# wangkepfe/Real-Time-Ray-Tracing

Hardware: AMD Instinct MI355X
Metric: Mray/s + ms/frame at 1080p 4spp (1/2/4/8 GPU); LBVH build ms (higher is better)
Workload: dtype f32; 1 GPU; BASELINE config 3: 1920x1080, 4 spp path trace + SVGF denoise + auto-exposure/tone map, per-frame LBVH rebuild; width=1920, height=1080, spp=4

## Files before the change

### include/rtx_amd.h

```cpp
#ifndef RTX_AMD_H
#define RTX_AMD_H

#include <stddef.h>
#include <stdint.h>

#ifdef __cplusplus
extern "C" {
#endif

#define RT_OK 0
#define RT_ERR_ARG (-1)
#define RT_ERR_HIP (-2)
#define RT_ERR_IO (-3)
#define RT_ERR_STATE (-4)
#define RT_ERR_NO_DEVICE (-5)
#define RT_ERR_DEVICE (-6)

typedef struct rt_context rt_context;


int rt_create(int screen_width, int screen_height, const char* config_toml, rt_context** out);

int rt_init(rt_context* ctx);

// ... 175 lines not shown
    float emission[3];
    float ior;
    float alpha;
    float f0[3];
} rt_material;
int rt_default_material(uint32_t id, rt_material* out);
int rt_set_materials(rt_context* ctx, uint32_t first_id, uint32_t count, const rt_material* m);
int rt_get_materials(const rt_context* ctx, uint32_t first_id, uint32_t count, rt_material* out);
int rt_reset_materials(rt_context* ctx);

int rt_trace_primary(rt_context* ctx, int frame_num, int with_detail);

int rt_path_trace(rt_context* ctx, int frame_num, int with_detail);

int rt_denoise_post(rt_context* ctx, int frame_num, int with_hdr);

int rt_get_ray_count(rt_context* ctx, uint64_t* rays, int reset);

#define RT_OWN_STREAM ((void*)(intptr_t)-1)
#define RT_STREAM_OFF ((void*)(intptr_t)-2)
int rt_set_stream(rt_context* ctx, void* stream);

#define RT_GBUFFER_SETS 4
#define RT_BUF_SET1 0x100
#define RT_BUF_SET2 0x200
#define RT_BUF_SET3 0x300
int rt_set_post_stream(rt_context* ctx, void* stream);

int rt_set_gather_stream(rt_context* ctx, void* stream);

typedef struct rt_strip_exchange {
    int32_t frameNum;
    int32_t rowBegin, rowEnd;
    int32_t historySet;
    int32_t gbufferSet;
    int32_t stripLocal;
} rt_strip_exchange;
#define RT_HOOK_HISTOGRAM 0
#define RT_HOOK_ROWS 1
#define RT_HOOK_GBUFFERS 2
typedef int (*rt_collective_fn)(void* arg, int stage, void* stream, const rt_strip_exchange* x);
int rt_set_collective_hook(rt_context* ctx, rt_collective_fn fn, void* arg);
int rt_set_hook_stages(rt_context* ctx, uint32_t stage_mask);

int rt_bind_buffer(rt_context* ctx, int name, void* device_ptr, size_t bytes);

int rt_sync(rt_context* ctx);

int rt_time_stage(rt_context* ctx, int stage, int iters, float* total_ms);

int rt_time_mesh_set(rt_context* ctx, int iters, float* parts_ms);

int rt_debug_pk_math(int fn, const float* x, float y, float c, float* out_pk, float* out_scalar, size_t n);

int rt_time_path_trace_kernels(rt_context* ctx, int iters, float* kernel_ms, int n);

int rt_time_frame_kernels(rt_context* ctx, int first_frame, int iters, float* kernel_ms, int n);

int rt_frame_marks_begin(rt_context* ctx, int frames, uint32_t kernel_mask);
int rt_frame_marks_read(rt_context* ctx, float* kernel_ms, int n, int* frames_recorded);

enum rt_array_name {
    RT_ARR_VERTICES = 0,
    RT_ARR_INDICES = 1,
    RT_ARR_NORMALS = 2,
    RT_ARR_TRI_POS = 3,
    RT_ARR_AABBS = 4,
    RT_ARR_MORTON = 5,
    RT_ARR_REORDER = 6,
    RT_ARR_NODES = 7,
    RT_ARR_TLAS_AABBS = 8,
    RT_ARR_TLAS_MORTON = 9,
    RT_ARR_TLAS_REORDER = 10,
    RT_ARR_TLAS_NODES = 11,
    RT_ARR_TLAS_SCENE_AABB = 12,
    RT_ARR_BATCH_SCENE_AABBS = 13,
    RT_ARR_HITS = 14,
    RT_ARR_HIT_NORMALS = 15,
    RT_ARR_HIT_FAKE_NORMALS = 16,
    RT_ARR_HIT_STATS = 17,
    RT_ARR_TRI_NRM = 18,
    RT_ARR_RAYS = 19,
    RT_ARR_SKY_PDF = 20,
    RT_ARR_SKY_CDF = 21,
    RT_ARR_SUN_PDF = 22,
    RT_ARR_SUN_CDF = 23,
    RT_ARR_SUN_DIR = 24,
    RT_ARR_HISTOGRAM = 25,
    RT_ARR_EXPOSURE = 26,
    RT_ARR_COLOR4 = 27,
    RT_ARR_COLOR16 = 28,
    RT_ARR_COLOR64 = 29,
    RT_ARR_RGBA8 = 30,
    RT_ARR_PT_QUEUE = 32,
    RT_ARR_PT_Q3_ORIGINS = 33,
    RT_ARR_PT_Q3_DIRS = 34,
    RT_ARR_PT_Q4_ORIGINS = 35,
    RT_ARR_PT_Q4_DIRS = 36,
    RT_ARR_PT_STATS = 31,
    RT_ARR_TEX_ALBEDO_AO = 37,
    RT_ARR_TEX_NORMAL_ROUGHNESS = 38,
    RT_ARR_TEX_HEIGHT = 39,
    RT_ARR_HDR = 40,
    RT_ARR_BVH_ARENA = 41,
    RT_ARR_TRI_MATERIALS = 42,
    RT_ARR_ADJ_OFFSETS = 43,
// ... 28 lines not shown
```

### real-time-ray-tracing_amd/csrc/bvh_kernels.h

```cpp
#pragma once
#include <hip/hip_runtime.h>
#include <stdint.h>

constexpr int kStatusTlasTimeout = 0;
constexpr int kStatusTlasTimeoutBuild = 1;
constexpr int kStatusMeshBadIndices = 2;
constexpr int kStatusMatUndeclared = 3;

struct BvhBuildParams {
    const float* vertices;
    const float* normals;
    const uint32_t* indices;
    uint32_t triCount;
    uint32_t triCountPadded;
    uint32_t batchCount;
    float4* triPos;
    float4* triNrm;
    float* aabbs;
    float* batchSceneAabbs;
    uint32_t* morton;
    uint32_t* reorder;
    void* nodes;
    float* tlasAabbs;
    float* tlasSceneAabb;
    uint32_t* tlasMorton;
    uint32_t* tlasReorder;
    void* tlasNodes;
    uint32_t* counter;
    uint32_t threads;
    uint32_t cus;
    uint32_t* status;
    uint64_t waitTicks;
    uint32_t skipPublish;
    uint32_t buildSeq;
};

struct TraceCamera {
    float pos[3];
    float adjustedFront[3], adjustedLeft[3], adjustedUp[3];
    float apertureLeft[3], apertureUp[3];
    float invRes[2];
};

constexpr uint32_t kRowBlock = 16;
__host__ __device__ inline uint32_t row_of(uint32_t y0, uint32_t nStrips, uint32_t strip, uint32_t yl) {
    return y0 + ((yl / kRowBlock) * nStrips + strip) * kRowBlock + yl % kRowBlock;
}
__host__ __device__ inline uint32_t local_row(uint32_t y0, uint32_t nStrips, uint32_t y) {
    const uint32_t r = y - y0;
    return (r / kRowBlock / nStrips) * kRowBlock + r % kRowBlock;
}
inline uint32_t strip_row_count(uint32_t height, uint32_t nStrips, uint32_t strip) {
    uint32_t n = 0;
    for (uint32_t b = strip; b * kRowBlock < height; b += nStrips) {
        const uint32_t lo = b * kRowBlock, hi = lo + kRowBlock < height ? lo + kRowBlock : height;
        n += hi - lo;
    }
    return n;
}

constexpr uint32_t kDenoiseBlock = 64;
inline bool denoise_rows(uint32_t height, uint32_t nStrips, uint32_t strip, uint32_t& a, uint32_t& b) {
    const uint32_t nb = (height + kDenoiseBlock - 1) / kDenoiseBlock;
    if (nStrips < 1 || strip >= nStrips || nb < nStrips) return false;
    const uint32_t b0 = (uint32_t)((uint64_t)strip * nb / nStrips), b1 = (uint32_t)((uint64_t)(strip + 1) * nb / nStrips);
    a = b0 * kDenoiseBlock;
    b = b1 * kDenoiseBlock < height ? b1 * kDenoiseBlock : height;
    return true;
}

constexpr uint32_t kGbufHaloTiles = 5;
inline void gbuffer_rows(uint32_t height, uint32_t a, uint32_t b, uint32_t& lo, uint32_t& hi) {
    const uint32_t t0 = a / 16, t1 = (b + 15) / 16;
    lo = t0 > kGbufHaloTiles ? (t0 - kGbufHaloTiles) * 16 : 0;
    hi = (t1 + kGbufHaloTiles) * 16 < height ? (t1 + kGbufHaloTiles) * 16 : height;
}

struct TracePrimaryParams {
    TraceCamera cam;
    uint32_t width, height;
    uint32_t y0, rows;
    uint32_t nStrips, strip;
    int frameNum;
    const uint8_t* bluenoise;
    const float4* triPos;
    const float4* triNrm;
    const void* nodes;
    const void* tlasNodes;
    float4* hitOut;
    float4* normalOut;
    float4* fakeNormalOut;
    uint32_t* statsOut;
};

struct GeomUpdateParams {
    const float* src;
    uint32_t first, count;
    float* vertices;
    float* normals;
    const uint32_t* indices;
    const uint32_t* cornerSlot;
    const uint32_t* adjOffsets;
    float* contrib;
    uint32_t nverts, triCountPadded;
    float* prevVerts;
};

struct GeomDispParams {
    const float* vertices;
    const float* prevVerts;
    const uint32_t* indices;
    float4* triDisp;
    uint32_t triCountPadded;
};

constexpr uint32_t kMeshSortThreads = 512;
constexpr uint32_t kMeshTilesMax = 256;
inline uint32_t mesh_tile_len(uint32_t corners) {
    const uint32_t per = (corners + kMeshTilesMax - 1) / kMeshTilesMax;
    return (per + kMeshSortThreads - 1) / kMeshSortThreads * kMeshSortThreads;
}
struct MeshSetParams {
    const uint32_t* srcIndices;
    uint32_t triCount, triCountPadded, nverts;
    uint32_t* indices;
    uint32_t* adjOffsets;
    uint32_t* adjCorner;
    uint32_t* cornerSlot;
    uint32_t* keys[2];
    uint32_t* vals[2];
    uint32_t* table;
    uint32_t* badCount;
    uint32_t* status;
};
extern "C" hipError_t rtk_launch_mesh_set(const MeshSetParams* p, hipStream_t stream, hipEvent_t afterIngest);

extern "C" hipError_t rtk_launch_geometry_update(const GeomUpdateParams* p, hipStream_t stream);
// ... 7 lines not shown
```

### real-time-ray-tracing_amd/csrc/context.cpp

```cpp
#include "context.h"

#include <dlfcn.h>
#include <stdio.h>
#include <string.h>

#include <algorithm>
#include <chrono>
#include <cmath>
#include <fstream>
#include <sstream>

#include "gaussian_tables.h"
#include "mat_kernels.h"
#include "rtmath.h"
#include "toml_lite.h"

namespace {

thread_local std::string g_createError;

void default_params(rt_params& p) {
    p.sky.needRegenerate = 1;
    p.sky.timeOfDay = 0.25f;
    p.sky.sunAxisAngle = 45.0f;
// ... 1131 lines not shown
    }
    if (!ctx->dMatTable) {
        if (int rc = dalloc(ctx, &ctx->dMatTable, 256 * sizeof(MatRecord))) return rc;
    }
    HIP_TRY(ctx, hipMemcpy(ctx->dMatTable, recs.data(), 256 * sizeof(MatRecord), hipMemcpyHostToDevice));
    ctx->matHost.swap(next);
    ctx->matCustom = true;
    ctx->matEmits = emits;
    ++ctx->matSerial;
    return RT_OK;
}

int rt_get_materials(const rt_context* ctx, uint32_t first_id, uint32_t count, rt_material* out) {
    if (!ctx || !out) return RT_ERR_ARG;
    if (count == 0u || (uint64_t)first_id + (uint64_t)count > 256u) return RT_ERR_ARG;
    for (uint32_t k = 0; k < count; ++k) {
        if (ctx->matCustom) out[k] = ctx->matHost[first_id + k];
        else (void)rt_default_material(first_id + k, &out[k]);
    }
    return RT_OK;
}

int rt_reset_materials(rt_context* ctx) {
    if (!ctx) return RT_ERR_ARG;
    if (!ctx->inited) { ctx->err = "rt_reset_materials before rt_init"; return RT_ERR_STATE; }
    if (int rc = sync_streams(ctx, false)) return rc;
    ctx->matCustom = false;
    ctx->matEmits = false;
    ++ctx->matSerial;
    return RT_OK;
}

int wait_bvh(rt_context* ctx) {
    if (ctx->buildOnSide[ctx->bvhSet])
        HIP_TRY(ctx, hipStreamWaitEvent(ctx->stream, ctx->buildDone[ctx->bvhSet], 0));
    return RT_OK;
}

int rt_trace_primary(rt_context* ctx, int frame_num, int with_detail) {
    if (!ctx) return RT_ERR_ARG;
    if (!ctx->inited) { ctx->err = "rt_trace_primary before rt_init"; return RT_ERR_STATE; }
    HostCamera hc;
    rt_camera_update(ctx->camera, ctx->renderW, ctx->renderH, hc);
    TracePrimaryParams p;
    p.cam = rt_trace_camera(hc);
    p.width = (uint32_t)ctx->renderW;
    p.height = (uint32_t)ctx->renderH;
    p.y0 = (uint32_t)ctx->stripY0;
    p.rows = (uint32_t)ctx->stripRows;
    p.nStrips = (uint32_t)ctx->stripCount;
    p.strip = (uint32_t)ctx->stripIndex;
    p.frameNum = frame_num;
    p.bluenoise = ctx->dBlueNoise;
    p.triPos = ctx->dTriPos;
    p.triNrm = ctx->dTriNrm;
    p.nodes = ctx->dNodes;
    p.tlasNodes = ctx->dTlasNodes;
    p.hitOut = ctx->dHits;
    p.normalOut = with_detail ? ctx->dHitNrm : nullptr;
    p.fakeNormalOut = with_detail ? ctx->dHitFake : nullptr;
    p.statsOut = with_detail ? ctx->dHitStats : nullptr;
    if (int rc = wait_bvh(ctx)) return rc;
    HIP_TRY(ctx, rtk_launch_trace_primary(&p, ctx->stream));
    return RT_OK;
}

int rt_sync(rt_context* ctx) {
    if (!ctx) return RT_ERR_ARG;
    if (!ctx->inited) return RT_OK;
    return sync_streams(ctx);
}

int rt_draw_frame_internal(rt_context* ctx);

int rt_time_stage(rt_context* ctx, int stage, int iters, float* total_ms) {
    if (!ctx || !total_ms || iters < 1) return RT_ERR_ARG;
    if (!ctx->inited) { ctx->err = "rt_time_stage before rt_init"; return RT_ERR_STATE; }
    if (ctx->postStream) {
        void* post = ctx->postStream;
        int rc = rt_set_post_stream(ctx, nullptr);
        if (rc == RT_OK) rc = rt_time_stage(ctx, stage, iters, total_ms);
        const int rc2 = rt_set_post_stream(ctx, post);
        return rc != RT_OK ? rc : rc2;
    }
    const MeshChange same{ctx->dIdxStage, ctx->mesh.triCount, ctx->nv};
    if (stage == 5 || stage == 6) {
        int rc = sync_streams(ctx, false);
        if (rc == RT_OK) rc = vertex_stage(ctx);
        if (rc != RT_OK) return rc;
        HIP_TRY(ctx, hipMemcpy(ctx->dVertStage, ctx->dVerts, (size_t)ctx->nv * 12, hipMemcpyDeviceToDevice));
        if (stage == 6)
            HIP_TRY(ctx, hipMemcpy(ctx->dIdxStage, ctx->dIdx, (size_t)ctx->mesh.triCount * 12, hipMemcpyDeviceToDevice));
        HIP_TRY(ctx, hipDeviceSynchronize());
    }
    HIP_TRY(ctx, hipEventRecord(ctx->ev0, ctx->stream));
    for (int i = 0; i < iters; ++i) {
        int rc = RT_OK;
        if (stage == 0) rc = rt_build_bvh(ctx);
        else if (stage == 5) rc = enqueue_vertex_update(ctx, ctx->dVertStage, 0, ctx->nv, nullptr, true, false);
        else if (stage == 6) rc = enqueue_vertex_update(ctx, ctx->dVertStage, 0, ctx->nv, nullptr, true, false, &same);
        else if (stage == 1) rc = rt_trace_primary(ctx, 1 + i, 0);
        else if (stage == 2) rc = rt_path_trace(ctx, 1 + i, 0);
        else if (stage == 3) {
            const int f = ctx->nextFrame++;
            if ((rc = rt_build_bvh(ctx)) == RT_OK && (rc = rt_path_trace(ctx, f, 0)) == RT_OK)
                rc = rt_denoise_post(ctx, f, 0);
// ... 305 lines not shown
```

### real-time-ray-tracing_amd/csrc/context.h

```cpp
#pragma once
#include <hip/hip_runtime.h>
#include <stdint.h>

#include <string>
#include <vector>

#include "../../include/rtx_amd.h"
#include "bvh_kernels.h"
#include "frame_kernels.h"
#include "scene_gen.h"
#include "soil_textures.h"

struct HostCamera {
    float pos[3], dir[3], left[3], up[3];
    float yaw, pitch, focal, aperture;
    float res[2], invRes[2], fov[2], tanHalfFov[2];
    float adjustedLeft[3], adjustedUp[3], adjustedFront[3], apertureLeft[3], apertureUp[3];
};

inline size_t arena_bytes(size_t B, size_t NP) { return (B * 1024 + B + NP) * 64; }

struct BvhBufs {
    float4* triPos = nullptr;
    float4* triNrm = nullptr;
    float* aabbs = nullptr;
    float* batchScene = nullptr;
    uint32_t* morton = nullptr;
    uint32_t* reorder = nullptr;
    void* nodes = nullptr;
    float* tlasAabbs = nullptr;
    float* tlasScene = nullptr;
    uint32_t* tlasMorton = nullptr;
    uint32_t* tlasReorder = nullptr;
    void* tlasNodes = nullptr;
    uint32_t* counter = nullptr;
    float4* triDisp = nullptr;
    uint32_t triCount = 0, triCountPadded = 0, B = 0;
    uint64_t meshSerial = 0;
};

#ifndef RTX_GB_SETS
#define RTX_GB_SETS RT_GBUFFER_SETS
#endif
constexpr int kGbSets = RTX_GB_SETS;

constexpr int kMatPool = 4;

struct FrameResources {
    bool ready = false;
    float* solar = nullptr;
    float* limb = nullptr;
    float* cie = nullptr;
    float4* sky = nullptr;
    float* skyPdf = nullptr;
    float* skyCdf = nullptr;
    float4* sun = nullptr;
    float* sunPdf = nullptr;
    float* sunCdf = nullptr;
    float* scanSums = nullptr;
    float* skyTree = nullptr;
    float* sunTree = nullptr;
    float* lightSel = nullptr;
    bool skyValid = false;
    rt_sky_params lastSky{};
    float sunDir[3] = {0, 1, 0};
    float cosThetaMax = 1.0f, sunArea = 0.0f;
    uint2* texAlbedo = nullptr;
    uint2* texNormal = nullptr;
    uint16_t* texHeight = nullptr;
    uint2* gColor[kGbSets] = {};
    uint2* gNormal[kGbSets] = {};
    uint2* gAlbedo[kGbSets] = {};
    uint16_t* gDepth[kGbSets] = {};
    uint32_t* gMotion[kGbSets] = {};
    int gbSet = 0;
    bool setInFlight[kGbSets] = {};
    uint2* color = nullptr;
    uint2* normal = nullptr;
    uint2* albedo = nullptr;
    uint16_t* depth = nullptr;
    uint32_t* motion = nullptr;
    uint32_t* rays = nullptr;
    uint4* ptStats = nullptr;
    unsigned long long* rayCounter = nullptr;
    PtWorkspace ws{};
    float4* camHit0Rec[kGbSets] = {};
    float* camHit0Err[kGbSets] = {};
    uint32_t* camSurface[kGbSets] = {};
    uint32_t* camCount[kGbSets] = {};
    uint32_t* lastCounters = nullptr;
    uint32_t* syncCount[3] = {};
    int syncIdx = 0;
    bool syncZeroed[3] = {};
    struct Spec {
        bool valid = false;
        bool shade = false;
        int block = 0;
        uint64_t epoch = 0;
        uint64_t matSerial = 0;
        PathTraceParams p{};
    } spec;
    bool specReady = false;
    bool gbBound = false;
    unsigned long long* specRayCounter = nullptr;
    int specCounts = 0;
    bool camInFlight[kGbSets] = {};
    PtQueue camQ3[kGbSets] = {}, camQ4[kGbSets] = {};
    float4* camHitRec[kGbSets] = {};
    float* camHitErr[kGbSets] = {};
    float4* camPathL[kGbSets] = {};
    uint32_t* camPending[kGbSets] = {};
    uint32_t* camShade3[kGbSets] = {};
    int lastSlot = 0;
    unsigned long long* q3Host = nullptr;
// ... 261 lines not shown
```

### real-time-ray-tracing_amd/csrc/debug_math.hip

```cpp
#include <hip/hip_runtime.h>

#include "rtmath_pk.h"
#include "rtx_amd.h"

namespace {
__global__ __launch_bounds__(256) void k_debug_pk(int fn, const float* x, float y, float c, float* outPk,
                                                  float* outScalar, size_t n) {
    const size_t i = (size_t)blockIdx.x * 256 + threadIdx.x;
    if (i >= n) return;
    const size_t j = (i ^ 1) < n ? (i ^ 1) : i;
    const rtpk::F2 v = {x[i], x[j]};
    float pk = 0.0f, sc = 0.0f;
    if (fn == 0) {
        pk = rtpk::pow_pos2(v, y, rtpk::pow_y_odd(y)).x;
        sc = rt_powf(x[i], y);
    } else if (fn == 1) {
        pk = rtpk::expf2(v).x;
        sc = rt_expf(x[i]);
    } else {
        pk = rtpk::div_rcp2(v, y, c).x;
        sc = rt_div_rcp(x[i], y, c);
    }
    outPk[i] = pk;
    outScalar[i] = sc;
}
}

extern "C" int rt_debug_pk_math(int fn, const float* x, float y, float c, float* out_pk, float* out_scalar, size_t n) {
    if (!x || !out_pk || !out_scalar || fn < 0 || fn > 2) return RT_ERR_ARG;
    if (fn == 0 && !(y > 0.0f && y < __builtin_inff())) return RT_ERR_ARG;
    if (n == 0) return RT_OK;
    hipLaunchKernelGGL(k_debug_pk, dim3((unsigned)((n + 255) / 256)), dim3(256), 0, 0, fn, x, y, c, out_pk, out_scalar, n);
    if (hipGetLastError() != hipSuccess || hipDeviceSynchronize() != hipSuccess) return RT_ERR_HIP;
    return RT_OK;
}
```

### real-time-ray-tracing_amd/csrc/frame.cpp

```cpp
#include <math.h>
#include <stdlib.h>
#include <string.h>

#include <chrono>
#include <fstream>
#include <utility>
#include <vector>

#include "context.h"
#include "rtmath.h"

namespace {

constexpr float kPi = 3.1415926535897932384626422832795028841971f;
constexpr float kTwoPi = 6.2831853071795864769252867665590057683943f;
constexpr float kPiOver180 = 0.01745329251f;

struct V3 { float x, y, z; };
V3 v3(float x, float y, float z) { return V3{x, y, z}; }
V3 operator+(V3 a, V3 b) { return v3(a.x + b.x, a.y + b.y, a.z + b.z); }
V3 operator*(V3 a, float s) { return v3(a.x * s, a.y * s, a.z * s); }
V3 operator*(float s, V3 a) { return v3(a.x * s, a.y * s, a.z * s); }
V3 operator-(V3 a) { return v3(-a.x, -a.y, -a.z); }
float dop(float a, float b, float c, float d) {
// ... 17 lines not shown
    const float n = sqrtf(v.x * v.x + v.y * v.y + v.z * v.z);
    return v3(v.x / n, v.y / n, v.z / n);
}

struct Quat { V3 v; float w; };
Quat qmul(const Quat& p, const Quat& q) { return Quat{p.w * q.v + q.w * p.v + cross(p.v, q.v), p.w * q.w - dot(p.v, q.v)}; }

V3 sun_direction(float timeOfDay, float sunAxisAngle) {
    const V3 axis = normalize(v3(0.0f, rt_cosf(sunAxisAngle * kPiOver180), rt_sinf(sunAxisAngle * kPiOver180)));
    const float angle = fmodf(timeOfDay * kPi, kTwoPi);
    const V3 v = cross(v3(0.0f, 1.0f, 0.0f), axis);
    const Quat q{normalize(axis) * rt_sinf(angle / 2), rt_cosf(angle / 2)};
    const Quat r = qmul(qmul(q, Quat{v, 0.0f}), Quat{-q.v, q.w});
    return normalize(r.v);
}

float fitting(const float* m, float s, int i) {
    return (rt_powf(1.0f - s, 5.0f) * m[i] + 5.0f * rt_powf(1.0f - s, 4.0f) * s * m[i + 9] +
            10.0f * rt_powf(1.0f - s, 3.0f) * rt_powf(s, 2.0f) * m[i + 18] +
            10.0f * rt_powf(1.0f - s, 2.0f) * rt_powf(s, 3.0f) * m[i + 27] +
            5.0f * (1.0f - s) * rt_powf(s, 4.0f) * m[i + 36] + rt_powf(s, 5.0f) * m[i + 45]);
}
float fitting2(const float* m, float s) {
    return (rt_powf(1.0f - s, 5.0f) * m[0] + 5.0f * rt_powf(1.0f - s, 4.0f) * s * m[1] +
            10.0f * rt_powf(1.0f - s, 3.0f) * rt_powf(s, 2.0f) * m[2] +
            10.0f * rt_powf(1.0f - s, 2.0f) * rt_powf(s, 3.0f) * m[3] + 5.0f * (1.0f - s) * rt_powf(s, 4.0f) * m[4] +
            rt_powf(s, 5.0f) * m[5]);
}

struct SkyTablesHost {
    std::vector<float> skyDataSets, skyDataSetsRad, solar, limb, cieX, cieY, cieZ;
};
SkyTablesHost g_tables;

bool load_sky_tables(const std::string& path, SkyTablesHost& t, std::string& err) {
    std::ifstream f(path, std::ios::binary);
    if (!f) { err = "cannot read " + path; return false; }
    uint32_t count = 0;
    f.read((char*)&count, 4);
    if (count != 7) { err = "bad sky table file " + path; return false; }
    uint32_t len[7];
    f.read((char*)len, sizeof(len));
    const uint32_t expect[7] = {540, 60, 1800, 60, 10, 10, 10};
    std::vector<float>* dst[7] = {&t.skyDataSets, &t.skyDataSetsRad, &t.solar, &t.limb, &t.cieX, &t.cieY, &t.cieZ};
    for (int i = 0; i < 7; ++i) {
        if (len[i] != expect[i]) { err = "bad sky table sizes in " + path; return false; }
        dst[i]->resize(len[i]);
        f.read((char*)dst[i]->data(), len[i] * 4);
    }
    if (!f) { err = "truncated " + path; return false; }
    return true;
}

bool sky_params_equal(const rt_sky_params& a, const rt_sky_params& b) {
    return a.timeOfDay == b.timeOfDay && a.sunAxisAngle == b.sunAxisAngle && a.skyScalar == b.skyScalar &&
           a.sunScalar == b.sunScalar && a.sunAngle == b.sunAngle;
}

int update_sky(rt_context* ctx) {
    FrameResources& fr = ctx->fr;
    rt_sky_params& sp = ctx->params.sky;
    const V3 sunDir = sun_direction(sp.timeOfDay, sp.sunAxisAngle);
    fr.sunDir[0] = sunDir.x; fr.sunDir[1] = sunDir.y; fr.sunDir[2] = sunDir.z;
    if (fr.skyValid && !sp.needRegenerate && sky_params_equal(sp, fr.lastSky)) return RT_OK;
    if (fr.spec.valid) HIP_TRY(ctx, hipStreamWaitEvent(ctx->stream, ctx->specDone, 0));
    if (ctx->postStream) {
        const int rc = sync_streams(ctx, false);
        if (rc != RT_OK) return rc;
    }
    sp.sunScalar = sp.sunScalar > 0.00001f ? sp.sunScalar : 0.00001f;
    sp.skyScalar = sp.skyScalar > 0.00001f ? sp.skyScalar : 0.00001f;
    sp.sunAngle = sp.sunAngle > 0.51f ? sp.sunAngle : 0.51f;
    SkyGenParams p;
    memcpy(p.sunDir, fr.sunDir, 12);
    p.skyScalar = sp.skyScalar;
    p.sunScalar = sp.sunScalar;
    p.sunAngle = sp.sunAngle;
    const float elevation = rt_acosf(sunDir.y);
    const float se = rt_powf(elevation / (kPi / 2.0f), (1.0f / 3.0f));
    for (int ch = 0; ch < 10; ++ch) {
        for (int i = 0; i < 9; ++i) p.st.configs[ch * 9 + i] = fitting(g_tables.skyDataSets.data() + ch * 54, se, i);
        p.st.radiances[ch] = fitting2(g_tables.skyDataSetsRad.data() + ch * 6, se);
    }
    const float sunRadius = sp.sunAngle * kPi / 180.0f / 2.0f;
    p.cosThetaMax = rt_cosf(sunRadius);
    p.solar = fr.solar;
    p.limb = fr.limb;
    p.cie = fr.cie;
    p.skyBuffer = fr.sky;
    p.skyPdf = fr.skyPdf;
    p.skyCdf = fr.skyCdf;
    p.sunBuffer = fr.sun;
    p.sunPdf = fr.sunPdf;
    p.sunCdf = fr.sunCdf;
    p.scanSums = fr.scanSums;
    p.skyTree = fr.skyTree;
    p.sunTree = fr.sunTree;
    p.lightSel = fr.lightSel;
    HIP_TRY(ctx, rtk_launch_sky(&p, ctx->stream));
    if (ctx->postStream) HIP_TRY(ctx, hipStreamSynchronize(ctx->stream));
    fr.sunArea = rt_powf(rt_tanf(sunRadius), 2.0f) * kPi;
    fr.cosThetaMax = p.cosThetaMax;
    fr.skyValid = true;
    sp.needRegenerate = 0;
    fr.lastSky = sp;
    return RT_OK;
}

float dop_host(float a, float b, float c, float d) {
    const float cd = c * d;
    const float err = fmaf(-c, d, cd);
    const float dp = fmaf(a, b, -cd);
    return dp + err;
}
void sun_frame(const float n[3], float t[3], float b[3]) {
    float w[3] = {1.0f, 0.0f, 0.0f};
    if (fabsf(n[0]) > 0.707f) { w[0] = 0.0f; w[1] = 1.0f; }
    auto cross = [](const float* a, const float* c, float* r) {
        r[0] = dop_host(a[1], c[2], a[2], c[1]);
        r[1] = dop_host(a[2], c[0], a[0], c[2]);
        r[2] = dop_host(a[0], c[1], a[1], c[0]);
    };
    cross(n, w, t);
    cross(n, t, b);
}

HistCamera hist_of(const HostCamera& c) {
    HistCamera h;
    memcpy(h.pos, c.pos, 12);
    memcpy(h.left, c.left, 12);
    memcpy(h.up, c.up, 12);
    memcpy(h.dir, c.dir, 12);
    return h;
}

}

void select_gbuffers(FrameResources& fr) {
    const int k = fr.gbSet;
    if (fr.renderColor == fr.color) fr.renderColor = fr.gColor[k];
    fr.color = fr.gColor[k];
    fr.normal = fr.gNormal[k];
    fr.albedo = fr.gAlbedo[k];
    fr.depth = fr.gDepth[k];
    fr.motion = fr.gMotion[k];
}

bool strip_local_denoise(const rt_context* ctx, uint32_t& a, uint32_t& b) {
    const rt_render_pass_settings& ps = ctx->params.pass;
    const uint32_t H = (uint32_t)ctx->renderH;
    a = 0;
// ... 152 lines not shown
}

float frame_delta(rt_context* ctx) {
    FrameResources& fr = ctx->fr;
    if (fr.drawDt >= 0.0f) {
        const float d = fr.drawDt;
        fr.drawDt = -1.0f;
        return d;
    }
    if (ctx->deltaMs > 0.0f) return ctx->deltaMs;
    const double now = std::chrono::duration<double>(std::chrono::steady_clock::now().time_since_epoch()).count();
    const float dt = fr.lastDrawTime < 0 ? 1000.0f / 60.0f : (float)((now - fr.lastDrawTime) * 1000.0);
    fr.lastDrawTime = now;
    return dt;
}

void update_dynamic_resolution(rt_context* ctx, float dt) {
    if (!(dt > 0.0f)) return;
    const float hi = 1000.0f / (ctx->targetFps - 2), lo = 1000.0f / (ctx->targetFps + 2);
    int w = ctx->renderW;
    if (hi < dt || lo > dt) {
        const float ratio = sqrtf((1000.0f / ctx->targetFps) / dt);
        w = (int)((float)w * ratio);
    }
    w = w + ((w % 16 < 8) ? (-w % 16) : (16 - w % 16));
    w = w < ctx->minWidth ? ctx->minWidth : w > ctx->maxWidth ? ctx->maxWidth : w;
    int h = (w / 16) * 9;
    if (h > ctx->maxHeight) h = ctx->maxHeight;
    ctx->renderW = w;
    ctx->renderH = h;
    ctx->stripRows = h;
}

int rt_frame_init(rt_context* ctx) {
    FrameResources& fr = ctx->fr;
    std::string err;
    if (g_tables.solar.empty()) {
        SkyTablesHost t;
        if (!load_sky_tables(rt_data_dir() + "/sky_tables.bin", t, err)) { ctx->err = err; return RT_ERR_IO; }
        g_tables = std::move(t);
    }
    int rc;
#define ALLOC(p, bytes) if ((rc = dalloc(ctx, &(p), (bytes))) != RT_OK) return rc
    ALLOC(fr.solar, 1800 * 4);
    ALLOC(fr.limb, 60 * 4);
    ALLOC(fr.cie, 30 * 4);
    ALLOC(fr.sky, (size_t)kSkySize * 16);
    ALLOC(fr.skyPdf, (size_t)kSkySize * 4);
    ALLOC(fr.skyCdf, (size_t)kSkySize * 4);
    ALLOC(fr.sun, (size_t)kSunSize * 16);
    ALLOC(fr.sunPdf, (size_t)kSunSize * 4);
    ALLOC(fr.sunCdf, (size_t)kSunSize * 4);
    ALLOC(fr.scanSums, 512 * 4);
    ALLOC(fr.skyTree, (size_t)kSkyTreeNodes * 4);
    ALLOC(fr.sunTree, (size_t)kSunTreeNodes * 4);
    ALLOC(fr.lightSel, 16);
    ALLOC(fr.texAlbedo, (size_t)kTexTexels * 8);
    ALLOC(fr.texNormal, (size_t)kTexTexels * 8);
    ALLOC(fr.texHeight, (size_t)kTexTexels * 2);
    HIP_TRY(ctx, hipMemset(fr.texHeight, 0, (size_t)kTexTexels * 2));
    const size_t P = (size_t)ctx->renderW * ctx->renderH;
    ALLOC(fr.color, P * 8);
    ALLOC(fr.normal, P * 8);
    ALLOC(fr.albedo, P * 8);
    ALLOC(fr.depth, P * 2);
    ALLOC(fr.motion, P * 4);
    fr.gColor[0] = fr.color;
    fr.gNormal[0] = fr.normal;
    fr.gAlbedo[0] = fr.albedo;
    fr.gDepth[0] = fr.depth;
    fr.gMotion[0] = fr.motion;
    ALLOC(fr.rays, P * 4);
    ALLOC(fr.ptStats, P * 16);
    ALLOC(fr.rayCounter, (size_t)kRayCounterSlots * kRayCounterStride * 8);
    {
        const size_t cap = (size_t)ctx->renderW * ctx->stripRows * ctx->spp;
        if (cap >= (1ull << 31)) { ctx->err = "strip x spp too large for the path-trace queues"; return RT_ERR_ARG; }
        PtWorkspace& ws = fr.ws;
        ws.cap = (uint32_t)cap;
        ALLOC(ws.hit0Rec, cap * 16);
        ALLOC(ws.hit0Err, cap * 4);
        for (PtQueue* q : {&ws.q3, &ws.q4}) {
            ALLOC(q->rayO, cap * 16);
            ALLOC(q->rayD, cap * 16);
            ALLOC(q->st0, cap * 16);
            ALLOC(q->st1, cap * 16);
            ALLOC(q->st2, cap * 16);
        }
        ALLOC(ws.hitRec, cap * 16);
        ALLOC(ws.hitErr, cap * 4);
        ALLOC(ws.pathL, cap * 16);
        if (ctx->tune.resumeSplit > 0) ALLOC(fr.camShade3[0], cap * 4);
        ALLOC(ws.pending, (size_t)ctx->renderW * ctx->stripRows * 4);
        ALLOC(ws.surface, (size_t)ctx->renderW * ctx->stripRows * 4);
        ALLOC(fr.camCount[0], kWsCounterWords * 4);
        ALLOC(fr.syncCount[1], kWsCounterWords * 4);
        ALLOC(fr.syncCount[2], kWsCounterWords * 4);
        fr.syncCount[0] = fr.camCount[0];
        fr.camQ3[0] = ws.q3;
        fr.camQ4[0] = ws.q4;
        fr.camHitRec[0] = ws.hitRec;
        fr.camHitErr[0] = ws.hitErr;
        fr.camPathL[0] = ws.pathL;
        fr.camPending[0] = ws.pending;
        fr.camHit0Rec[0] = ws.hit0Rec;
        fr.camHit0Err[0] = ws.hit0Err;
        fr.camSurface[0] = ws.surface;
        ws.counters = fr.camCount[0];
        ws.fetch = ws.counters + 64;
// ... 126 lines not shown
    if (queues) {
        for (PtQueue* q : {&fr.camQ3[k], &fr.camQ4[k]}) {
            ALLOC(q->rayO, cap * 16);
            ALLOC(q->rayD, cap * 16);
            ALLOC(q->st0, cap * 16);
            ALLOC(q->st1, cap * 16);
            ALLOC(q->st2, cap * 16);
        }
        ALLOC(fr.camHitRec[k], cap * 16);
        ALLOC(fr.camHitErr[k], cap * 4);
        ALLOC(fr.camPathL[k], cap * 16);
        ALLOC(fr.camPending[k], strip * 4);
        if (ctx->tune.resumeSplit > 0) ALLOC(fr.camShade3[k], cap * 4);
    }
#undef ALLOC
    return rc;
}

int fill_pt_params(const rt_context* ctx, int frame_num, int with_detail, const HostCamera& hc, int g,
                   PathTraceParams& p) {
    const FrameResources& fr = ctx->fr;
    memset(&p, 0, sizeof p);
    p.cam = rt_trace_camera(hc);
    p.tanHalfFov[0] = hc.tanHalfFov[0];
    p.tanHalfFov[1] = hc.tanHalfFov[1];
    p.res[0] = hc.res[0];
    p.res[1] = hc.res[1];
    p.halfRes[0] = hc.res[0] / 2;
    p.halfRes[1] = hc.res[1] / 2;
    p.hist = fr.hist;
    p.width = (uint32_t)ctx->renderW;
    p.height = (uint32_t)ctx->renderH;
    p.y0 = (uint32_t)ctx->stripY0;
    p.rows = (uint32_t)ctx->stripRows;
    p.nStrips = (uint32_t)ctx->stripCount;
    p.strip = (uint32_t)ctx->stripIndex;
    p.frameNum = frame_num;
    p.spp = (uint32_t)ctx->spp;
    p.invSpp = (ctx->spp & (ctx->spp - 1)) == 0 ? 1.0f / (float)ctx->spp : 0.0f;
    p.materialOverride = ctx->materialOverride;
    p.triCount = ctx->bvh[ctx->bvhSet].triCount;
    p.bluenoise = ctx->dBlueNoise;
    p.triPos = ctx->dTriPos;
    p.triNrm = ctx->dTriNrm;
    p.triDisp = ctx->dispValid[ctx->bvhSet] && !ctx->dispTraced[ctx->bvhSet] ? ctx->bvh[ctx->bvhSet].triDisp : nullptr;
    p.nodes = ctx->dNodes;
    p.tlasNodes = ctx->dTlasNodes;
    p.texAlbedo = fr.texAlbedo;
    p.texNormal = fr.texNormal;
    p.skyBuffer = fr.sky;
    p.sunBuffer = fr.sun;
    p.skyCdf = fr.skyCdf;
    p.sunCdf = fr.sunCdf;
    p.skyTree = fr.skyTree;
    p.sunTree = fr.sunTree;
    p.lightSel = fr.lightSel;
    memcpy(p.sunDir, fr.sunDir, 12);
    p.cosThetaMax = fr.cosThetaMax;
    p.oneMinusCosThetaMax = 1.0f - fr.cosThetaMax;
    sun_frame(fr.sunDir, p.sunT, p.sunB);
    p.colorOut = fr.gColor[g];
    p.normalOut = fr.gNormal[g];
    p.albedoOut = fr.gAlbedo[g];
    p.depthOut = fr.gDepth[g];
    p.motionOut = fr.gMotion[g];
    p.raysOut = with_detail ? fr.rays : nullptr;
    p.statsOut = with_detail ? fr.ptStats : nullptr;
    p.rayCounter = fr.rayCounter;
    p.ws = fr.ws;
    p.ws.hit0Rec = fr.camHit0Rec[g];
    p.ws.hit0Err = fr.camHit0Err[g];
    p.ws.surface = fr.camSurface[g];
    p.ws.counters = fr.camCount[g];
    p.ws.fetch = p.ws.counters + 64;
    const int qs = fr.camQ3[g].rayO ? g : 0;
    p.ws.q3 = fr.camQ3[qs];
    p.ws.q4 = fr.camQ4[qs];
    p.ws.hitRec = fr.camHitRec[qs];
    p.ws.hitErr = fr.camHitErr[qs];
    p.ws.pathL = fr.camPathL[qs];
    p.ws.pending = fr.camPending[qs];
    p.ws.hitRec4 = p.ws.hitRec;
    p.ws.hitErr4 = p.ws.hitErr;
    p.ws.shade3 = fr.camShade3[qs];
    {
        const int m = ctx->materialOverride;
        uint32_t classes = ctx->dTriMat ? ctx->triMatClasses : 0u;
        if (m >= 0) {
            const uint8_t id = (uint8_t)(m > 255 ? 255 : m);
            (void)rt_material_classes(&id, 1, &classes);
        }
        p.triMat = m >= 0 ? nullptr : ctx->dTriMat;
        p.ws.glossy = (classes & RT_MAT_CLASS_GLOSSY) != 0u;
        p.ws.microfacet = (classes & RT_MAT_CLASS_MICROFACET) != 0u;
        p.matTable = ctx->matCustom ? reinterpret_cast<const float4*>(ctx->dMatTable) : nullptr;
        if (p.matTable) p.ws.glossy = p.ws.microfacet = 1;
        p.ws.closest4 = p.matTable && ctx->matEmits ? 1 : 0;
    }
    return qs;
}

bool spec_on(const rt_context* ctx) {
    return ctx->tune.syncSpec && ctx->fr.specReady && !ctx->postStream && ctx->stripCount == 1 && !ctx->fr.gbBound;
}

bool spec_matches(const PathTraceParams& a, uint64_t epochA, uint64_t matA, const PathTraceParams& b, uint64_t epochB,
                  uint64_t matB) {
    if (epochA != epochB) return false;
    if (matA != matB) return false;
// ... 838 lines not shown
    HIP_TRY(ctx, hipMemsetAsync(fr.ws.counters, 0, kWsCounterWords * sizeof(uint32_t), ctx->stream));
    HIP_TRY(ctx, hipMemcpyAsync(fr.ws.counters + kCntQ3, &n, 4, hipMemcpyHostToDevice, ctx->stream));
    HIP_TRY(ctx, hipEventRecord(ctx->ev0, ctx->stream));
    HIP_TRY(ctx, rtk_launch_trace_queue(&p, 3, ctx->stream));
    HIP_TRY(ctx, hipEventRecord(ctx->ev1, ctx->stream));
    HIP_TRY(ctx, hipMemcpyAsync(hits, fr.ws.hitRec, (size_t)n * 16, hipMemcpyDeviceToHost, ctx->stream));
    if (iters) HIP_TRY(ctx, hipMemcpyAsync(iters, p.ws.itersOut, (size_t)n * 4, hipMemcpyDeviceToHost, ctx->stream));
    HIP_TRY(ctx, hipStreamSynchronize(ctx->stream));
    if (kernel_ms) HIP_TRY(ctx, hipEventElapsedTime(kernel_ms, ctx->ev0, ctx->ev1));
    return RT_OK;
}

int rt_trace_rays_device(rt_context* ctx, const rt_ray_query* q) {
    if (!ctx || !q) return RT_ERR_ARG;
    const char* bad = nullptr;
    if (q->org_stride < 3u || q->dir_stride < 3u) bad = "strides are in floats and at least 3";
    else if (q->n > RT_QUERY_MAX_RAYS) bad = "more rays than RT_QUERY_MAX_RAYS";
    else if ((q->flags & ~RT_QUERY_ANY_HIT) != 0u) bad = "unknown flags";
    else if (q->n > 0u && (!q->org || !q->dir || !q->hits)) bad = "org, dir and hits must not be NULL";
    else if (((uintptr_t)q->hits & 15u) != 0) bad = "hits must be 16-byte aligned";
    else if ((((uintptr_t)q->org | (uintptr_t)q->dir | (uintptr_t)q->iters) & 3u) != 0) bad = "org, dir and iters must be 4-byte aligned";
    if (bad) { ctx->err = std::string("rt_trace_rays_device: ") + bad; return RT_ERR_ARG; }
    if (!ctx->inited) { ctx->err = "rt_trace_rays_device before rt_init"; return RT_ERR_STATE; }
    hipStream_t s = ctx->stream;
    if (q->n > 0u) {
        if (q->ready_event) HIP_TRY(ctx, hipStreamWaitEvent(s, (hipEvent_t)q->ready_event, 0));
        if (int rc = wait_bvh(ctx)) return rc;
        RayQueryParams p;
        p.nodes = ctx->dNodes;
        p.tlasNodes = ctx->dTlasNodes;
        p.triPos = ctx->dTriPos;
        p.org = q->org;
        p.dir = q->dir;
        p.orgStride = q->org_stride;
        p.dirStride = q->dir_stride;
        p.n = q->n;
        p.hits = reinterpret_cast<float4*>(q->hits);
        p.iters = q->iters;
        p.fetch = ctx->queryFetch;
        HIP_TRY(ctx, hipMemsetAsync(ctx->queryFetch, 0, 512, s));
        HIP_TRY(ctx, rtk_launch_trace_rays(&p, ctx->fr.ws.traceBlocks, (q->flags & RT_QUERY_ANY_HIT) != 0u, s));
        const int k = ctx->bvhSet;
        if (ctx->postStream) {
            HIP_TRY(ctx, hipEventRecord(ctx->bvhFree[k], s));
            ctx->bvhInFlight[k] = true;
        } else {
            HIP_TRY(ctx, hipEventRecord(ctx->queryDone[k], s));
            ctx->queryInFlight[k] = true;
        }
    }
    if (q->done_event) HIP_TRY(ctx, hipEventRecord((hipEvent_t)q->done_event, s));
    return RT_OK;
}
```

### real-time-ray-tracing_amd/csrc/frame_kernels.h

```cpp
#pragma once
#include <hip/hip_runtime.h>
#include <stdint.h>

#include "bvh_kernels.h"
#include "rtx_amd.h"

constexpr int kSkyW = 512, kSkyH = 256, kSkySize = kSkyW * kSkyH;
constexpr int kSunW = 32, kSunH = 32, kSunSize = kSunW * kSunH;
constexpr int kSkyScanBlock = 256, kSunScanBlock = 32;
constexpr int kTexLevels = 11, kTexSize = 1024;

static_assert((kTexSize & (kTexSize - 1)) == 0 && kTexSize <= 16384, "power-of-two texture size");
__host__ __device__ constexpr uint32_t tex_level_offset(int l) {
    return 4u * ((uint32_t)(kTexSize * kTexSize) - (uint32_t)(kTexSize >> l) * (uint32_t)(kTexSize >> l)) / 3u;
}
constexpr uint32_t kTexTexels = tex_level_offset(kTexLevels);

struct SkyState {
    float configs[90];
    float radiances[10];
};

struct SkyGenParams {
    float sunDir[3];
    float skyScalar, sunScalar, sunAngle;
    float cosThetaMax;
    SkyState st;
    const float* solar;
    const float* limb;
    const float* cie;
    float4* skyBuffer;
    float* skyPdf;
    float* skyCdf;
    float4* sunBuffer;
    float* sunPdf;
    float* sunCdf;
    float* scanSums;
    float* skyTree;
    float* sunTree;
    float* lightSel;
};

constexpr int kSkyTreeNodes = 4096, kSunTreeNodes = 1024;

struct HistCamera { float pos[3], left[3], up[3], dir[3]; };

constexpr uint32_t kQShadowFlag = 1u;

__host__ __device__ inline bool q3_shades(uint32_t flags, uint32_t hitIdxBits) {
    return (flags & kQShadowFlag) == 0u && (int32_t)hitIdxBits >= 0;
}

struct PtQueue {
    float4* rayO;
    float4* rayD;
    float4* st0;
    float4* st1;
    float4* st2;
};

enum PtCounter : int { kCntQ3 = 0, kCntQ4 = 1, kCntFetch3 = 2, kCntFetch4 = 3, kCntPending = 4, kCntResume3 = 5,
                       kCntResume4 = 6, kCntResolve = 7, kCntMaxIter3 = 8, kCntMaxIter4 = 9, kCntError = 10,
                       kCntSurface = 11, kCntVisCam = 12, kCntTstCam = 13, kCntVisShade = 14, kCntTstShade = 15,
                       kCntVisQ3 = 16, kCntTstQ3 = 17, kCntVisQ4 = 18, kCntTstQ4 = 19, kCntDiffShade = 20,
                       kCntDiffRes3 = 21, kCntCulledCam = 22, kCntShade3 = 23, kCntSlots = 24 };
constexpr int kWsCounterWords = 64 + 3 * 8 * 16;
constexpr uint32_t kChainMaxQ3 = 1u << 20;

struct PtWorkspace {
    float4* hit0Rec;
    float* hit0Err;
    PtQueue q3, q4;
    float4* hitRec;
    float* hitErr;
    float4* hitRec4 = nullptr;
    float* hitErr4 = nullptr;
    uint32_t* shade3 = nullptr;
    float4* pathL;
    uint32_t* pending;
    uint32_t* surface;
    uint32_t* counters;
    uint32_t* fetch;
    uint32_t cap;
    uint32_t persistBlocks;
    int shadeClaim = 0;
    uint32_t shadeBlocksPerCu = 0;
    uint32_t cus = 256;
    uint32_t traceBlocks;
    uint32_t trace3ShortBlocks = 0;
    uint32_t trace4Blocks;
    int glossy;
    int microfacet;
    int chain = 1;
    int closest4 = 0;
    uint32_t* itersOut = nullptr;
    unsigned long long* q3HostOut = nullptr;
    uint32_t q3Tag = 0;
    uint32_t* zeroNext = nullptr;
    int countersZeroed = 0;
};

enum class PtBouncePlan { chain, split, unsplit };
inline PtBouncePlan pt_bounce_plan(const PtWorkspace& ws) {
    if (ws.chain && !ws.glossy && !ws.microfacet) return PtBouncePlan::chain;
    return ws.shade3 && !ws.glossy ? PtBouncePlan::split : PtBouncePlan::unsplit;
}

constexpr int kRayCounterSlots = 256, kRayCounterStride = 16;

struct PathTraceParams {
    TraceCamera cam;
    float tanHalfFov[2];
    float res[2];
    float halfRes[2];
    HistCamera hist;
    uint32_t width, height;
    uint32_t y0, rows;
    uint32_t nStrips, strip;
    int frameNum;
    uint32_t spp;
    float invSpp;
    int materialOverride;
    uint32_t triCount;
    const uint8_t* bluenoise;
    const float4* triPos;
    const float4* triNrm;
    const void* nodes;
    const void* tlasNodes;
    const uint2* texAlbedo;
    const uint2* texNormal;
    const float4* skyBuffer;
    const float4* sunBuffer;
    const float* skyCdf;
    const float* sunCdf;
    const float* skyTree;
    const float* sunTree;
    const float* lightSel;
    float sunDir[3];
    float sunT[3], sunB[3];
    float cosThetaMax;
    float oneMinusCosThetaMax;
    uint2* colorOut;
    uint2* normalOut;
    uint2* albedoOut;
    uint16_t* depthOut;
    uint32_t* motionOut;
    uint32_t* raysOut;
    uint4* statsOut;
    unsigned long long* rayCounter;
    PtWorkspace ws;
    const float4* triDisp;
    const uint8_t* triMat;
    const float4* matTable;
};

constexpr int kMatRecVecs = 4;
struct alignas(16) MatRecord {
    float color[3];
    uint32_t typeFlags;
    float f0[3];
    float alpha;
    float emission[3];
    float ior;
    float pad[4];
};
static_assert(sizeof(MatRecord) == 16 * kMatRecVecs, "four 16-byte vectors");

struct DenoisePostParams {
    uint32_t W, H;
    uint32_t Ws, Hs;
    uint32_t histW, histH;
    int frameNum;
    float deltaTime;
    int temporal, localSpatial, visualize, wideSpatial, temporal2;
    int postProcess, downScale, histogramOn, autoExposure, sharpen, tonemap;
    int bloom, lensFlare;
    int toneMappingType;
    float sunPos[2];
    int sunUv[2];
    uint2* bloom4;
    uint2* bloom16;
    float gain, fixedExposure, maxWhite, gamma;
    rt_denoising_params dn;
    uint2* colorA;
    uint2* colorB;
    uint2* normal;
    const uint2* albedo;
    uint16_t* depth;
    const uint32_t* motion;
    uint2* accum;
    uint2* accumAlt;
    uint2* histColor;
    uint2* histColorOut;
    uint16_t* histDepth;
    uint16_t* noise8;
    uint16_t* noise16;
    uint2* c4;
    uint2* c16;
    uint2* c64;
    uint32_t* histogram;
    float* exposure;
    uint2* scaledA;
    uint2* scaledB;
    uint32_t* rgba;
    uint32_t rgbaPitch;
    const uint8_t* bluenoise;
    float4* hdrOut;
    uint2* finalColor;
    uint2* finalScaled;
    int stripLocal;
    uint32_t rowA, rowB;
    int histOutSet;
    int gbSet;
    uint32_t* rgbaTarget;
    uint32_t rgbaTargetPitch;
    int ty0, ty1;
    int cty0, cty1;
    uint32_t* chainCounter;
    int exposureDone;
    int histDepthInTemporal;
    uint2* svgfOut;
    int histDepthDone;
    uint32_t* tileList;
    uint32_t tileCap;
    int tileParity;
    int listUsed;
    int listSplit;
    int listFold;
    float rcpDepth[3];
    int rcpDepthOk;
    hipEvent_t* marks;
};
constexpr int kDnKernels = 8;

extern "C" hipError_t rtk_denoise_post(DenoisePostParams* p, hipStream_t stream);
extern "C" hipError_t rtk_denoise_phase(DenoisePostParams* p, hipStream_t stream, int phase);
extern "C" hipError_t rtk_hdr_out(const uint2* color, float4* hdr, size_t n, hipStream_t stream);

extern "C" hipError_t rtk_launch_sky(const SkyGenParams* p, hipStream_t stream);
extern "C" hipError_t rtk_launch_mipgen(uint16_t* chain, int size, int levels, int channels, hipStream_t stream);
extern "C" hipError_t rtk_launch_scan(const float* in, float* out, float* sums, int size, int blockSize,
                                      hipStream_t stream);
extern "C" hipError_t rtk_launch_scan_ex(const float* in, float* out, float* sums, int size, int blockSize,
                                         int postfix, hipStream_t stream);
constexpr int kPtKernels = 7;
constexpr int kFrameKernels = kPtKernels + kDnKernels;
struct PtLaunchHook {
    hipError_t (*fn)(void* arg, int kernel);
    void* arg;
};
struct PtLeanFork {
    hipStream_t stream;
    hipEvent_t traced, done;
};
extern "C" hipError_t rtk_launch_pt_camera(const PathTraceParams* p, hipStream_t stream, hipEvent_t* marks);
extern "C" hipError_t rtk_launch_pt_rest(const PathTraceParams* p, hipStream_t stream, hipEvent_t* marks,
                                         const PtLaunchHook* hook, const PtLeanFork* fork);
extern "C" hipError_t rtk_launch_pt_shade(const PathTraceParams* p, hipStream_t stream, hipEvent_t* marks);
extern "C" hipError_t rtk_fold_ray_counts(unsigned long long* dst, unsigned long long* src, hipStream_t stream);
extern "C" hipError_t rtk_launch_pt_rest_after_shade(const PathTraceParams* p, hipStream_t stream, hipEvent_t* marks,
                                                     const PtLaunchHook* hook, const PtLeanFork* fork);
extern "C" int rtk_trace_queue_blocks_per_cu();
extern "C" hipError_t rtk_launch_trace_queue(const PathTraceParams* p, int step, hipStream_t stream);

struct RayQueryParams {
    const void* nodes;
    const void* tlasNodes;
    const float4* triPos;
    const float* org;
    const float* dir;
    uint32_t orgStride, dirStride;
    uint32_t n;
    float4* hits;
    uint32_t* iters;
    uint32_t* fetch;
};
extern "C" hipError_t rtk_launch_trace_rays(const RayQueryParams* p, uint32_t maxBlocks, int anyHit, hipStream_t stream);
```

### real-time-ray-tracing_amd/csrc/pathtrace.hip

```cpp
#include "frame_kernels.h"
#include "pt_common.h"
#include "queue_fetch.h"
#include "shade.h"
#include "traverse.h"

using namespace rtd;

namespace {

constexpr uint32_t kQShadow = kQShadowFlag;
constexpr int kQSampleShift = 1;
constexpr int kQLightShift = 16;

struct RayState {
    F3 orig, dir, pos, normal, fakeNormal, albedo, centerRaydir;
    int matId, matType, lightIdx, objectIdx;
    bool isRayIntoSurface, hitLight, hit, isDiffuse, isHitProcessed, isOccluded, isShadowRay;
    float offset, normalDotRayDir, depth, rayConeWidth, rayConeSpread;
};

struct PathCtx {
    const PathTraceParams& P;
    F3 sunDir;
    const uint32_t* sob;
    BnPixel bp;
    int frameIdx;
    uint32_t rays, visits, tests, diffuse;
    const float* skyTree = nullptr;
    const float* sunTree = nullptr;
};

RT_DEV PathCtx path_ctx(const PathTraceParams& P, const uint32_t* sob, const float* skyTree, const float* sunTree) {
    return PathCtx{P, f3(P.sunDir[0], P.sunDir[1], P.sunDir[2]), sob, BnPixel{0u, 0u}, 0, 0u, 0u, 0u, 0u, skyTree, sunTree};
}

RT_DEV void stage_cdf_trees(const PathTraceParams& P, float* sky, float* sun, int tid, int nthreads) {
    for (int i = tid; i < kSkyTreeNodes / 4; i += nthreads) reinterpret_cast<float4*>(sky)[i] = reinterpret_cast<const float4*>(P.skyTree)[i];
    for (int i = tid; i < kSunTreeNodes / 4; i += nthreads) reinterpret_cast<float4*>(sun)[i] = reinterpret_cast<const float4*>(P.sunTree)[i];
}

RT_DEV float rnd(const PathCtx& c, int k, int d) { return bn_value(c.sob, c.bp, c.frameIdx * 4 + k, d); }

struct PathVars {
    RayState rs;
    F3 beta0, beta1;
    float outDepth;
    uint32_t mask;
    F2 mv, sampleUv;
    F3 outNormal;
};

RT_DEV float4 mat_vec(const PathTraceParams& P, int id, int k) { return P.matTable[(id & 255) * kMatRecVecs + k]; }

template <bool kTab = false>
RT_DEV void update_material(const PathTraceParams& P, RayState& rs) {
    const bool inRange = rs.objectIdx >= 0 && rs.objectIdx < (int)P.triCount;
    int tableId = 3;
    if (P.triMat && inRange) tableId = (int)P.triMat[rs.objectIdx];
    const int id = P.materialOverride >= 0 ? P.materialOverride : inRange ? tableId : 6;
    int type;
    if constexpr (kTab) type = (int)(__float_as_uint(mat_vec(P, id, 0).w) & 0xFFu);
    else type = (id >= 0 && id < 10) ? mat_type(id) : PERFECT_REFLECTION;
    rs.matId = rs.hit ? id : 99999;
    rs.matType = rs.hit ? type : MAT_SKY;
    if (rs.isShadowRay) {
        if ((rs.matType == EMISSIVE && rs.lightIdx == rs.objectIdx) || (rs.matType == MAT_SKY && rs.lightIdx == kEnvLightId))
            rs.hitLight = true;
        else
            rs.isOccluded = true;
    } else {
        rs.hitLight = rs.matType == EMISSIVE || rs.matType == MAT_SKY;
    }
    rs.isDiffuse = (rs.matType == LAMBERTIAN) || (rs.matType == MICROFACET);
}

RT_DEV bool needs_trace(const RayState& rs) { return !(rs.hitLight || !rs.isHitProcessed || rs.isOccluded); }

template <bool kTab = false>
RT_DEV void apply_hit(const PathTraceParams& P, RayState& rs, const HitInfo& h) {
    rs.isHitProcessed = false;
    rs.offset = h.offset;
    rs.objectIdx = h.objectIdx;
    rs.pos = h.pos;
    rs.normal = h.normal;
    rs.fakeNormal = h.fakeNormal;
    rs.normalDotRayDir = h.ndr;
    rs.isRayIntoSurface = h.into;
    rs.hit = h.hit;
    rs.depth = h.t;
    if (rs.hit) rs.rayConeWidth += rs.rayConeSpread * h.t;
    update_material<kTab>(P, rs);
}

template <bool kTab = false>
// ... 36 lines not shown
RT_DEV void tri_plane(const PathTraceParams& P, F2 uv, float lod, F3 normal, F3 w, F3& alb, F3& nrm) {
    uv.x *= 0.5f;
    uv.y *= 0.5f;
    const F4 t0 = sample_lod(P.texAlbedo, uv, lod);
    __builtin_amdgcn_sched_barrier(0);
    alb = f3(rt_powf_div(t0.x, 2.2f), rt_powf_div(t0.y, 2.2f), rt_powf_div(t0.z, 2.2f));
    __builtin_amdgcn_sched_barrier(0);
    const F4 t1 = sample_lod(P.texNormal, uv, lod);
    const F3 n = f3(t1.x - 0.5f, t1.y - 0.5f, t1.z - 0.5f);
    const F3 u = cross(normal, w);
    const F3 v = cross(normal, u);
    nrm = normalize(u * n.x + v * n.y + normal * n.z);
}

template <bool kMF, bool kTab = false>
RT_DEV void diffuse(PathCtx& c, int bounce, RayState& rs, F3& beta) {
    if (rs.hitLight || !rs.isDiffuse || rs.isOccluded) return;
    const PathTraceParams& P = c.P;
    ++c.diffuse;
    rs.lightIdx = kDefaultLightId;
    rs.isHitProcessed = true;
    F3 normal = rs.fakeNormal;
    const F3 surfaceNormal = rs.normal;
    F3 albedo;
    bool flat = false;
    if constexpr (kTab) flat = ((__float_as_uint(mat_vec(P, rs.matId, 0).w) >> 8) & RT_MAT_FLAG_FLAT) != 0u;
    if (!flat) {
        const float lod = rt_log2f_div(rs.rayConeWidth * 0.5f * __builtin_sqrtf(1024.0f * 1024.0f + 1024.0f * 1024.0f));
        const float wx = surfaceNormal.x * surfaceNormal.x, wy = surfaceNormal.y * surfaceNormal.y,
                    wz = surfaceNormal.z * surfaceNormal.z;
        F3 accA = f3(0.0f), accN = f3(0.0f);
#pragma unroll 1
        for (int pl = 0; pl < 3; ++pl) {
            const F2 uv = pl == 0 ? F2{rs.pos.y, rs.pos.z} : pl == 1 ? F2{rs.pos.x, rs.pos.z} : F2{rs.pos.x, rs.pos.y};
            F3 wv;
            if (pl == 0) wv = fabsf(normal.y) > 0.999f ? f3(0, 0, 1) : f3(0, 1, 0);
            else if (pl == 1) wv = fabsf(normal.x) > 0.999f ? f3(0, 0, 1) : f3(1, 0, 0);
            else wv = fabsf(normal.y) > 0.999f ? f3(1, 0, 0) : f3(0, 1, 0);
            F3 a, n;
            tri_plane(P, uv, lod, normal, wv, a, n);
            const float wgt = pl == 0 ? wx : pl == 1 ? wy : wz;
            accA = pl == 0 ? a * wgt : accA + a * wgt;
            accN = pl == 0 ? n * wgt : accN + n * wgt;
        }
        albedo = accA;
        normal = normalize(accN);
        rs.fakeNormal = normal;
    }
    if constexpr (kTab) {
        const float4 m0 = mat_vec(P, rs.matId, 0);
        albedo = flat ? f3(m0.x, m0.y, m0.z) : albedo * f3(m0.x, m0.y, m0.z);
    }
    if (bounce == 0) rs.albedo = albedo * (1.0f + fabsf(dot(normal, rs.centerRaydir)));
    float r[4], r2[4];
#pragma unroll
    for (int d = 0; d < 4; ++d) {
        r[d] = rnd(c, 2 * bounce, d);
        r2[d] = rnd(c, 2 * bounce + 1, d);
    }
    const F3 rayDir = rs.dir;
    F3 lDir;
    float lPdf = 1.0f;
    int lIdx;
    sample_light(P, c.sunDir, lDir, lPdf, lIdx, r2[0], r2[1], c.skyTree, c.sunTree);
    F3 sDir, sBsdf, lBsdf, tmp;
    float sPdf = 0.0f;
    if (!kMF || rs.matType == LAMBERTIAN) {
        lambertian_sample(F2{r[0], r[1]}, sDir, normal);
        sBsdf = f3(div_pi(albedo.x), div_pi(albedo.y), div_pi(albedo.z));
        sPdf = div_pi(fmx(dot(sDir, normal), kSafeCos));
        lBsdf = sBsdf;
    } else {
        F3 F0 = mat_F0(rs.matId);
        float alpha = mat_alpha(rs.matId);
        if constexpr (kTab) {
            const float4 m1 = mat_vec(P, rs.matId, 1);
            F0 = f3(m1.x, m1.y, m1.z);
            alpha = m1.w;
        }
        const float alpha2 = alpha * alpha;
        const F3 sn = ggx_normal(F2{r[0], r[1]}, alpha2, normal);
        sDir = normalize(reflect3(rayDir, sn));
        if (dot(sDir, surfaceNormal) < 0.0f) {
            const F3 sn2 = ggx_normal(F2{r[2], r[3]}, alpha2, normal);
            sDir = normalize(reflect3(rayDir, sn2));
            if (dot(sDir, surfaceNormal) < 0.0f) sDir = normalize(reflect3(rayDir, normal));
        }
        float lsPdf;
        microfacet_terms(-rayDir, sDir, sn, normal, F0, albedo, alpha2, tmp, sBsdf, sPdf);
        microfacet_terms(-rayDir, lDir, normalize(lDir + -rayDir), normal, F0, albedo, alpha2, tmp, lBsdf, lsPdf);
    }
    if (isnan3(lBsdf)) lBsdf = f3(0.0f);
    if (isnan3(sBsdf)) sBsdf = f3(0.0f);
    if (sPdf != sPdf) sPdf = 0.0f;
    if (lPdf != lPdf) lPdf = 0.0f;
    const float ph = (sPdf * sPdf) / (sPdf * sPdf + lPdf * lPdf);
    const float minPdf = 1e-5f;
    if (r[3] < ph) {
        if (dot(rs.normal, sDir) < 0.0f) { rs.isOccluded = true; return; }
        const float cwi = fmx(kSafeCos, dot(sDir, normal));
        beta = sBsdf * cwi / fmx(sPdf, minPdf);
        rs.dir = sDir;
    } else {
        if (dot(rs.normal, lDir) < 0.0f) { rs.isOccluded = true; return; }
        const float cwi = fmx(kSafeCos, dot(lDir, normal));
        beta = lBsdf * cwi / fmx(lPdf, minPdf);
        rs.dir = lDir;
        rs.lightIdx = lIdx;
        rs.isShadowRay = true;
    }
    if (isnan3(beta)) beta = f3(0.0f);
    rs.orig = rs.pos + rs.offset * rs.normal;
}

RT_DEV float ray_cone_width(const PathTraceParams& P, int ix, int iy) {
    const F2 pc = {((float)ix + 0.5f) - P.halfRes[0], ((float)iy + 0.5f) - P.halfRes[1]};
    const F2 po = {copysignf(0.5f, pc.x), copysignf(0.5f, pc.y)};
    const F2 un = {(pc.x - po.x) * P.cam.invRes[0] * 2, (pc.y - po.y) * P.cam.invRes[1] * 2};
    const F2 uf = {(pc.x + po.x) * P.cam.invRes[0] * 2, (pc.y + po.y) * P.cam.invRes[1] * 2};
    const F2 pn = {un.x * P.tanHalfFov[0], un.y * P.tanHalfFov[1]};
    const F2 pf = {uf.x * P.tanHalfFov[0], uf.y * P.tanHalfFov[1]};
    const float an = rt_atanf(__builtin_sqrtf(pn.x * pn.x + pn.y * pn.y));
    const float af = rt_atanf(__builtin_sqrtf(pf.x * pf.x + pf.y * pf.y));
    return af - an;
}

RT_DEV void gbuffer_step0(const PathCtx& c, PathVars& v) {
    const RayState& rs = v.rs;
    v.outDepth = rs.depth;
    v.mask = (uint32_t)rs.matId & 0xFFFFu;
    F2 mv = {0.0f, 0.0f};
    if (rs.hit) {
        const PathTraceParams& P = c.P;
        const F3 d = rs.pos - load3(P.hist.pos);
        const F3 q = f3(dot(load3(P.hist.left), d), dot(load3(P.hist.up), d), dot(load3(P.hist.dir), d));
        const F2 s = {q.x / q.z, q.y / q.z};
        const F2 ndc = {s.x / P.tanHalfFov[0], s.y / P.tanHalfFov[1]};
        mv = F2{(0.5f - ndc.x * 0.5f) - v.sampleUv.x, (0.5f - ndc.y * 0.5f) - v.sampleUv.y};
    }
    v.mv = F2{mv.x + 0.5f, mv.y + 0.5f};
}

template <int kDeferFrom, bool kMF, bool kTab = false>
RT_DEV int run_path(PathCtx& c, PathVars& v, int k0, const HitInfo* hit, const SceneView& sc, uint2* stk) {
    RayState& rs = v.rs;
    if (hit) apply_hit<kTab>(c.P, rs, *hit);
#pragma unroll 1
    for (int k = k0; k < 5; ++k) {
        if ((k != k0 || !hit) && needs_trace(rs)) {
            if (k >= kDeferFrom) return k;
            ++c.rays;
// ... 81 lines not shown
    const uint32_t flags = (rs.isShadowRay ? kQShadow : 0u) | (s << kQSampleShift) |
                           ((uint32_t)rs.lightIdx << kQLightShift);
    q.rayO[slot] = make_float4(rs.orig.x, rs.orig.y, rs.orig.z, __uint_as_float(pixel));
    q.rayD[slot] = make_float4(rs.dir.x, rs.dir.y, rs.dir.z, __uint_as_float(flags));
    q.st0[slot] = make_float4(rs.albedo.x, rs.albedo.y, rs.albedo.z, rs.rayConeWidth);
    q.st1[slot] = make_float4(v.beta1.x, v.beta1.y, v.beta1.z, rs.rayConeSpread);
    q.st2[slot] = make_float4(v.beta0.x, v.beta0.y, v.beta0.z, 0.0f);
}

RT_DEV SceneView scene_of(const PathTraceParams& P) { return scene_view(P.nodes, P.tlasNodes, P.triPos, P.triNrm); }

template <bool kBits = false>
RT_DEV void add_rays(const PathTraceParams& P, unsigned long long* wgSlots, uint32_t rays, int w) {
    if (!P.rayCounter) return;
    uint32_t r = rays;
    if (kBits) {
        r = (uint32_t)__popcll(__ballot(rays != 0u));
    } else {
#pragma unroll
        for (int o = 32; o > 0; o >>= 1) r += __shfl_xor(r, o);
    }
    const bool lane0 = __lane_id() == 0;
    if (lane0) wgSlots[w] = r;
    __syncthreads();
    const uint32_t slot = (blockIdx.y * gridDim.x + blockIdx.x) % kRayCounterSlots;
    if (w == 0 && lane0)
        atomicAdd(&P.rayCounter[slot * kRayCounterStride], wgSlots[0] + wgSlots[1] + wgSlots[2] + wgSlots[3]);
}
template <bool kBits = false>
RT_DEV void add_rays(const PathTraceParams& P, unsigned long long* wgSlots, uint32_t rays) {
    add_rays<kBits>(P, wgSlots, rays, __builtin_amdgcn_readfirstlane((int)threadIdx.x >> 6));
}

RT_DEV void start_sample(PathCtx& c, PathVars& v, int x, int y, float coneSpread, F3 centerDir) {
    RayState& rs = v.rs;
    v.beta0 = f3(1.0f);
    v.beta1 = f3(1.0f);
    rs.hitLight = false;
    rs.lightIdx = kDefaultLightId;
    rs.isHitProcessed = true;
    rs.isOccluded = false;
    rs.isShadowRay = false;
    rs.isDiffuse = false;
    rs.hit = false;
    rs.matType = MAT_SKY;
    rs.matId = 0;
    rs.objectIdx = -1;
    rs.normal = f3(0.0f, -1.0f, 0.0f);
    rs.fakeNormal = f3(0.0f);
    rs.albedo = f3(1.0f);
    rs.rayConeWidth = 0.0f;
    rs.rayConeSpread = coneSpread;
    rs.centerRaydir = centerDir;
    generate_ray_jittered(c.P.cam, x, y, F2{rnd(c, 0, 0), rnd(c, 0, 1)}, F2{rnd(c, 0, 2), rnd(c, 0, 3)}, rs.orig,
                          rs.dir, v.sampleUv);
    v.outDepth = 0.0f;
    v.mask = 0u;
    v.mv = F2{0.0f, 0.0f};
    v.outNormal = f3(0.0f);
}

}

__host__ __device__ inline int cam_sample_waves(uint32_t spp) { return spp >= 4 ? 4 : (spp >= 2 ? 2 : 1); }
inline bool one_round(uint32_t spp) { return spp >= 1 && ((int)spp + cam_sample_waves(spp) - 1) / cam_sample_waves(spp) == 1; }

template <bool kOneRound, bool kStats>
__global__ __launch_bounds__(256, kOneRound ? 6 : 4) void k_pt_camera(PathTraceParams P) {
    constexpr int kCamLds = 10;
    __shared__ uint2 stk[kCamLds * 256];
    __shared__ uint32_t sob[256];
    __shared__ float4 fold[4][64];
    __shared__ uint32_t surf[4][64];
    __shared__ unsigned long long wgRays[4];
    const int tid = threadIdx.x, lane = tid & 63, w = tid >> 6;
    bn_stage_sobol(P.bluenoise, sob, tid, 256);
    __syncthreads();
    const int nSW = cam_sample_waves(P.spp);
    const int sw = w % nSW, g = w / nSW, tilesX = nSW == 4 ? 1 : 2;
    const int BW = 8 * tilesX, BH = nSW == 1 ? 16 : 8;
    const int x = blockIdx.x * BW + (g % tilesX) * 8 + (lane & 7);
    const int yl = blockIdx.y * BH + (g / tilesX) * 8 + (lane >> 3);
    const bool active = x < (int)P.width && yl < (int)P.rows;
    const int y = (int)row_of(P.y0, P.nStrips, P.strip, (uint32_t)yl);
    const uint32_t p = (uint32_t)y * P.width + (uint32_t)x;
    const uint32_t pl = (uint32_t)yl * P.width + (uint32_t)x;
    const size_t plane = (size_t)P.rows * P.width;
    const SceneView sc = scene_of(P);
    PathCtx c = path_ctx(P, sob, nullptr, nullptr);
    if (active) c.bp = bn_pixel(P.bluenoise, x, y);
    const int rounds = kOneRound ? 1 : ((int)P.spp + nSW - 1) / nSW;
    F3 L = f3(0.0f), A = f3(0.0f);
    bool anyHit = false;
    float4 rec = make_float4(0.0f, 0.0f, 0.0f, 0.0f);
    float recErr = 0.0f;
    uint32_t rays = 0, camV = 0, camT = 0, camCull = 0;
#pragma unroll 1
    for (int r = 0; r < rounds; ++r) {
        const int s = r * nSW + sw;
        float4 out = make_float4(0.0f, 0.0f, 0.0f, 0.0f);
        if (active && s < (int)P.spp) {
            c.frameIdx = (int)P.spp * (P.frameNum - 1) + 1 + s;
            F3 org, dir;
            F2 uv;
            generate_ray_jittered(P.cam, x, y, F2{rnd(c, 0, 0), rnd(c, 0, 1)}, F2{rnd(c, 0, 2), rnd(c, 0, 3)}, org,
                                  dir, uv);
            TravState st;
            if (root_surely_missed(sc, org, dir)) {
                trav_root_miss(st, sc.root);
                ++camCull;
            } else {
                TravRay tr;
                trav_setup(sc, org, dir, tr);
                trav_init(st, sc.root);
                DeepStack deep;
                TravRec trec;
                for (int it = 0; it < 1024; ++it)
                    if (trav_step<kCamLds, false, kStats>(sc, tr, st, trec, stk + tid, 256, &deep)) break;
            }
            ++rays;
            if (P.statsOut) {
                camV += st.visits;
                camT += st.tests;
            }
            rec = make_float4(st.t, __uint_as_float((uint32_t)st.hitIdx), st.hitU, st.hitV);
            recErr = st.hitErrT;
            if (rounds > 1) {
                P.ws.hit0Rec[(size_t)s * plane + pl] = rec;
                P.ws.hit0Err[(size_t)s * plane + pl] = recErr;
            }
            if (st.t < kRayMax) {
                out.w = 1.0f;
            } else {
                PathVars v;
                v.rs.dir = dir;
                v.rs.hitLight = true;
                v.rs.isOccluded = false;
                v.rs.matType = MAT_SKY;
                v.rs.albedo = f3(1.0f);
                v.beta0 = f3(1.0f);
                v.beta1 = f3(1.0f);
                const F3 Ls = finish(c, v);
                out = make_float4(Ls.x, Ls.y, Ls.z, 0.0f);
            }
        }
        fold[w][lane] = out;
        __syncthreads();
        if (sw == 0 && active) {
#pragma unroll 1
            for (int k = 0; k < nSW; ++k) {
                const int sk = r * nSW + k;
                if (sk >= (int)P.spp) break;
                const float4 o = fold[g * nSW + k][lane];
                anyHit = anyHit || o.w != 0.0f;
                if (P.spp == 1) {
                    L = f3(o.x, o.y, o.z);
                    A = f3(1.0f);
                } else {
                    L = L + f3(o.x, o.y, o.z);
// ... 42 lines not shown
    add_rays<kOneRound>(P, wgRays, rays);
}

struct ShadeClaim {
    uint32_t batches, partLen, drained, next;
    int home;
    bool dyn;
};
RT_DEV void claim_init(ShadeClaim& c, uint32_t batches, bool dyn) {
    c.batches = batches;
    c.partLen = (batches + kParts - 1) / kParts;
    c.drained = batches == 0u ? (1u << kParts) - 1u : 0u;
    c.home = (int)(blockIdx.x % kParts);
    c.dyn = dyn;
    c.next = blockIdx.x;
}
RT_DEV uint32_t claim_next(ShadeClaim& c, uint32_t* counters, uint32_t& slot) {
    if (!c.dyn) {
        const uint32_t b = c.next;
        c.next += gridDim.x;
        return b;
    }
    __syncthreads();
    if (threadIdx.x == 0) {
        uint32_t b = c.batches;
        while (c.drained != (1u << kParts) - 1u) {
            int part = c.home;
            while (c.drained & (1u << part)) part = (part + 1) % kParts;
            const uint32_t got = atomicAdd(&counters[part * 16], 1u);
            const uint32_t lo = (uint32_t)part * c.partLen;
            const uint32_t len = lo >= c.batches ? 0u : (c.batches - lo < c.partLen ? c.batches - lo : c.partLen);
            if (got < len) {
                b = lo + got;
                break;
            }
            c.drained |= 1u << part;
        }
        slot = b;
    }
    __syncthreads();
    return slot;
}

template <bool kGlossy, bool kMF, bool kOneRound, bool kTab = false>
#ifndef RTX_SHADE_WAVES
#define RTX_SHADE_WAVES 3
#endif
__global__ __launch_bounds__(256, (kGlossy || !kOneRound) ? 2 : RTX_SHADE_WAVES) void k_pt_shade0(PathTraceParams P) {
    __shared__ uint2 stk[kGlossy ? 17 * 256 : 1];
    __shared__ uint32_t sob[256];
    __shared__ float4 foldL[4][64];
    __shared__ float4 foldA[4][64];
    __shared__ unsigned long long wgRays[4];
    __shared__ __align__(16) float sSkyTree[kSkyTreeNodes];
    __shared__ __align__(16) float sSunTree[kSunTreeNodes];
    __shared__ uint32_t wgBatch;
    const int tid = threadIdx.x, lane = tid & 63, w = tid >> 6;
    const int wS = __builtin_amdgcn_readfirstlane(w);
    bn_stage_sobol(P.bluenoise, sob, tid, 256);
    stage_cdf_trees(P, sSkyTree, sSunTree, tid, 256);
    __syncthreads();
    const uint32_t n = P.ws.counters[kCntSurface];
    const int nSW = cam_sample_waves(P.spp), sw = w % nSW, g = w / nSW;
    const uint32_t perWg = 64u * (uint32_t)(4 / nSW);
    const int rounds = kOneRound ? 1 : ((int)P.spp + nSW - 1) / nSW;
    const SceneView sc = scene_of(P);
    const size_t plane = (size_t)P.rows * P.width;
    uint32_t raysWg = 0, shV = 0, shT = 0, shD = 0;
    ShadeClaim claim;
    claim_init(claim, (n + perWg - 1) / perWg, P.ws.shadeClaim != 0);
#pragma unroll 1
    for (uint32_t base; (base = claim_next(claim, P.ws.fetch + 2 * kParts * 16, wgBatch) * perWg) < n;) {
        const uint32_t i = base + (uint32_t)g * 64u + (uint32_t)lane;
        const bool active = i < n;
        const uint32_t pl = active ? P.ws.surface[i] : 0u;
        const int x = (int)(pl % P.width), yl = (int)(pl / P.width);
        const int y = (int)row_of(P.y0, P.nStrips, P.strip, (uint32_t)yl);
        const uint32_t p = (uint32_t)y * P.width + (uint32_t)x;
        PathCtx c = path_ctx(P, sob, sSkyTree, sSunTree);
        float coneSpread = 0.0f;
        F3 centerDir = f3(0.0f);
        if (active) {
            c.bp = bn_pixel(P.bluenoise, x, y);
            coneSpread = ray_cone_width(P, x, y);
            centerDir = center_dir(P.cam, x, y);
        }
        F3 L = f3(0.0f), A = f3(0.0f), L0s = f3(0.0f), A0s = f3(0.0f), N0 = f3(0.0f);
        float D0 = 0.0f;
        F2 M0 = {0.0f, 0.0f};
        uint32_t mask0 = 0u;
        int sd = -1;
#pragma unroll 1
        for (int r = 0; r < rounds; ++r) {
            const int s = r * nSW + sw;
            const bool run = active && s < (int)P.spp;
            PathVars v;
            int kd = 5;
            if (run) {
                c.frameIdx = (int)P.spp * (P.frameNum - 1) + 1 + s;
                start_sample(c, v, x, y, coneSpread, centerDir);
                const size_t q = (size_t)s * plane + pl;
                const float4 hr = P.ws.hit0Rec[q];
                HitInfo h;
                finalize_hit(sc, v.rs.orig, v.rs.dir, hr.x, (int)__float_as_uint(hr.y), hr.z, hr.w, P.ws.hit0Err[q],
                             h);
                static_assert(!kTab || kGlossy, "the table variant is the all-classes kernel's");
                if constexpr (kGlossy) kd = run_path<3, kMF, kTab>(c, v, 0, &h, sc, stk + tid);
                else kd = run_shade0_diffuse<kMF>(c, v, h);
                if (kd < 3) {
                    atomicAdd(&P.ws.counters[kCntError], 1u);
                    kd = 5;
                }
            }
            const uint32_t slot3 = wave_append(kd == 3, &P.ws.counters[kCntQ3]);
            const uint32_t slot4 = wave_append(kd == 4, &P.ws.counters[kCntQ4]);
            float4 outL = make_float4(0.0f, 0.0f, 0.0f, 0.0f), outA = outL;
            if (run) {
                outA = make_float4(v.rs.albedo.x, v.rs.albedo.y, v.rs.albedo.z, 0.0f);
                if (s == 0) {
                    N0 = v.outNormal;
                    D0 = v.outDepth;
                    M0 = v.mv;
                    mask0 = v.mask;
                }
                if (kd < 5) {
                    ++c.rays;
                    enqueue(kd == 3 ? P.ws.q3 : P.ws.q4, kd == 3 ? slot3 : slot4, v, p, (uint32_t)s);
                    outL.w = 1.0f;
                } else {
                    const F3 Ls = finish<kTab>(c, v);
                    outL = make_float4(Ls.x, Ls.y, Ls.z, 0.0f);
                }
// ... 36 lines not shown
            }
            if (N0.x != N0.x || N0.y != N0.y || N0.z != N0.z) N0 = f3(0.0f);
            if (D0 != D0) D0 = 0.0f;
            if (M0.x != M0.x || M0.y != M0.y) M0 = F2{0.0f, 0.0f};
            if (sd >= 0) {
                P.ws.pending[pslot] = pl | ((uint32_t)sd << 26);
                P.colorOut[p] = make_uint2(0u, mask0 << 16);
            } else {
                P.colorOut[p] = pack_h4(L.x, L.y, L.z, mask0);
            }
            P.normalOut[p] = pack_h4(N0.x, N0.y, N0.z, 0u);
            P.albedoOut[p] = pack_h4(A.x, A.y, A.z, 0u);
            P.depthOut[p] = rt_f2h(D0);
            P.motionOut[p] = (uint32_t)rt_f2h(M0.x) | ((uint32_t)rt_f2h(M0.y) << 16);
        }
        if (active && c.rays) {
            if (P.raysOut) atomicAdd(&P.raysOut[p], c.rays);
            if (P.statsOut) atomicAdd(&P.statsOut[p].x, c.rays);
        }
        if (active && P.statsOut) {
            if (c.visits) atomicAdd(&P.statsOut[p].y, c.visits);
            if (c.tests) atomicAdd(&P.statsOut[p].z, c.tests);
            if (c.diffuse) atomicAdd(&P.statsOut[p].w, c.diffuse);
            shV += c.visits;
            shT += c.tests;
            shD += c.diffuse;
        }
        raysWg += c.rays;
    }
    if (P.statsOut) {
        wave_add(shV, &P.ws.counters[kCntVisShade]);
        wave_add(shT, &P.ws.counters[kCntTstShade]);
        wave_add(shD, &P.ws.counters[kCntDiffShade]);
    }
    add_rays(P, wgRays, raysWg, wS);
}

__global__ __launch_bounds__(256) void k_pt_geom_motion(PathTraceParams P) {
    __shared__ uint32_t sob[256];
    const int tid = threadIdx.x;
    bn_stage_sobol(P.bluenoise, sob, tid, 256);
    __syncthreads();
    const uint32_t n = P.ws.counters[kCntSurface];
    const SceneView sc = scene_of(P);
#pragma unroll 1
    for (uint32_t i = blockIdx.x * 256u + (uint32_t)tid; i < n; i += gridDim.x * 256u) {
        const uint32_t pl = P.ws.surface[i];
        const float4 hr = P.ws.hit0Rec[pl];
        const int tri = (int)__float_as_uint(hr.y);
        if (!(hr.x < kRayMax) || tri < 0) continue;
        const int x = (int)(pl % P.width), yl = (int)(pl / P.width);
        const int y = (int)row_of(P.y0, P.nStrips, P.strip, (uint32_t)yl);
        const uint32_t p = (uint32_t)y * P.width + (uint32_t)x;
        PathCtx c = path_ctx(P, sob, nullptr, nullptr);
        c.bp = bn_pixel(P.bluenoise, x, y);
        c.frameIdx = (int)P.spp * (P.frameNum - 1) + 1;
        PathVars v;
        start_sample(c, v, x, y, 0.0f, f3(0.0f));
        HitInfo h;
        finalize_hit(sc, v.rs.orig, v.rs.dir, hr.x, tri, hr.z, hr.w, P.ws.hit0Err[pl], h);
        const F3 d1 = f3_of(P.triDisp[3 * tri]), d2 = f3_of(P.triDisp[3 * tri + 1]), d3 = f3_of(P.triDisp[3 * tri + 2]);
        v.rs.pos = h.pos - (d3 * (1.0f - hr.z - hr.w) + d1 * hr.z + d2 * hr.w);
        v.rs.hit = true;
        v.rs.depth = h.t;
        gbuffer_step0(c, v);
        F2 M = v.mv;
        if (M.x != M.x || M.y != M.y) M = F2{0.0f, 0.0f};
        P.motionOut[p] = (uint32_t)rt_f2h(M.x) | ((uint32_t)rt_f2h(M.y) << 16);
    }
}

template <int kStep, bool kMF, bool kTab = false>
RT_DEV int resume_diffuse(PathCtx& c, PathVars& v, const HitInfo& hit) {
    apply_hit<kTab>(c.P, v.rs, hit);
    if (kStep == 4) return 5;
    F3 beta = f3(1.0f);
    diffuse<kMF, kTab>(c, 1, v.rs, beta);
    v.beta0 = beta;
    return needs_trace(v.rs) ? 4 : 5;
}

RT_DEV void reload_entry(PathCtx& c, const PtQueue& q, const SceneView& sc, uint32_t i, float4 hr, float herr,
                         PathVars& v, uint32_t& p, uint32_t& s, HitInfo& h) {
    const PathTraceParams& P = c.P;
    const float4 o = q.rayO[i], d = q.rayD[i], s0 = q.st0[i], s1 = q.st1[i], s2 = q.st2[i];
    p = __float_as_uint(o.w);
    const uint32_t flags = __float_as_uint(d.w);
    s = (flags >> kQSampleShift) & 63u;
    const int x = (int)(p % P.width), y = (int)(p / P.width);
    c.bp = bn_pixel(P.bluenoise, x, y);
    c.frameIdx = (int)P.spp * (P.frameNum - 1) + 1 + (int)s;
    RayState& rs = v.rs;
    rs.orig = f3(o.x, o.y, o.z);
    rs.dir = f3(d.x, d.y, d.z);
    rs.isShadowRay = (flags & kQShadow) != 0u;
    rs.lightIdx = (int)(flags >> kQLightShift);
    rs.albedo = f3(s0.x, s0.y, s0.z);
    rs.rayConeWidth = s0.w;
    v.beta1 = f3(s1.x, s1.y, s1.z);
    rs.rayConeSpread = s1.w;
    v.beta0 = f3(s2.x, s2.y, s2.z);
    rs.hitLight = false;
    rs.isOccluded = false;
    rs.isHitProcessed = true;
    rs.isDiffuse = false;
    rs.centerRaydir = f3(0.0f);
    rs.matId = 0;
    rs.matType = MAT_SKY;
    finalize_hit(sc, rs.orig, rs.dir, hr.x, (int)__float_as_uint(hr.y), hr.z, hr.w, herr, h);
}

template <int kStep, bool kMF, bool kGlossy, bool kTab = false>
RT_DEV int resume_entry(PathCtx& c, const PtQueue& q, const SceneView& sc, uint32_t i, float4 hr, float herr,
                        PathVars& v, uint32_t& p, uint32_t& s) {
    HitInfo h;
    reload_entry(c, q, sc, i, hr, herr, v, p, s, h);
    if constexpr (kGlossy && kStep == 3) return run_path<0, kMF, kTab>(c, v, kStep, &h, sc, nullptr);
    else return resume_diffuse<kStep, kMF, kTab>(c, v, h);
}

template <bool kTab = false>
RT_DEV void store_path_L(const PathCtx& c, const PathVars& v, uint32_t p, uint32_t s) {
    const PathTraceParams& P = c.P;
    const F3 Ls = finish<kTab>(c, v);
    const uint32_t pl = local_row(P.y0, P.nStrips, p / P.width) * P.width + p % P.width;
    P.ws.pathL[(size_t)pl * P.spp + s] = make_float4(Ls.x, Ls.y, Ls.z, 0.0f);
}

template <bool kTab = false>
RT_DEV uint32_t finish_entry(PathCtx& c, const PathVars& v, bool active, int kd, uint32_t p, uint32_t s, uint32_t& rays,
                             uint32_t& rsD) {
    const PathTraceParams& P = c.P;
    const uint32_t slot = wave_append(kd == 4, &P.ws.counters[kCntQ4]);
    if (active) {
        if (kd < 5) {
            ++c.rays;
            enqueue(P.ws.q4, slot, v, p, s);
        } else {
            store_path_L<kTab>(c, v, p, s);
        }
        if (P.raysOut && c.rays) atomicAdd(&P.raysOut[p], c.rays);
        if (P.statsOut) {
            if (c.rays) atomicAdd(&P.statsOut[p].x, c.rays);
            if (c.diffuse) atomicAdd(&P.statsOut[p].w, c.diffuse);
            rsD += c.diffuse;
        }
        rays += c.rays;
    }
    return slot;
}

template <int kStep, bool kMF, bool kGlossy, bool kListed, bool kTab = false>
RT_DEV void resume_queue(const PathTraceParams& P) {
    static_assert(!kListed || (kStep == 3 && !kGlossy), "the shading list is queue 3's, kept without glossy tables");
    __shared__ uint32_t sob[256];
    __shared__ unsigned long long wgRays[4];
    __shared__ __align__(16) float sSkyTree[kStep == 3 ? kSkyTreeNodes : 4];
    __shared__ __align__(16) float sSunTree[kStep == 3 ? kSunTreeNodes : 4];
    const uint32_t n = P.ws.counters[kListed ? kCntShade3 : kStep == 3 ? kCntQ3 : kCntQ4];
    if (blockIdx.x * 256u >= n) return;
    const int tid = threadIdx.x;
    bn_stage_sobol(P.bluenoise, sob, tid, 256);
    if (kStep == 3) stage_cdf_trees(P, sSkyTree, sSunTree, tid, 256);
    __syncthreads();
    const PtQueue& q = kStep == 3 ? P.ws.q3 : P.ws.q4;
    const float4* hitRec = kStep == 3 ? P.ws.hitRec : P.ws.hitRec4;
    const float* hitErr = kStep == 3 ? P.ws.hitErr : P.ws.hitErr4;
    const SceneView sc = scene_of(P);
    uint32_t rays = 0, rsD = 0;
#pragma unroll 1
    for (uint32_t base = blockIdx.x * 256u; base < n; base += gridDim.x * 256u) {
        const uint32_t li = base + (uint32_t)tid;
        const bool active = li < n;
        PathCtx c = path_ctx(P, sob, sSkyTree, sSunTree);
        PathVars v;
        int kd = 5;
        uint32_t p = 0, s = 0;
        if (active) {
            const uint32_t i = kListed ? P.ws.shade3[li] : li;
            kd = resume_entry<kStep, kMF, kGlossy, kTab>(c, q, sc, i, hitRec[i], hitErr[i], v, p, s);
        }
        finish_entry<kTab>(c, v, active, kd, p, s, rays, rsD);
    }
    if (kStep == 3 && P.statsOut) wave_add(rsD, &P.ws.counters[kCntDiffRes3]);
    add_rays(P, wgRays, rays);
}

template <int kStep, bool kMF, bool kGlossy, bool kTab = false>
__global__ __launch_bounds__(256, kStep == 3 ? (kGlossy ? 2 : 3) : 4) void k_pt_resume(PathTraceParams P) {
    static_assert(!kTab || kStep == 4 || (kMF && kGlossy), "the table variant is the all-classes kernel's");
    resume_queue<kStep, kMF, kGlossy, false, kTab>(P);
}

template <bool kMF>
__global__ __launch_bounds__(256, 3) void k_pt_resume3_shade(PathTraceParams P) {
    resume_queue<3, kMF, false, true>(P);
}

__global__ __launch_bounds__(256) void k_pt_resume3_lean(PathTraceParams P) {
    const uint32_t n = P.ws.counters[kCntQ3];
    const SceneView sc = scene_of(P);
#pragma unroll 1
    for (uint32_t i = blockIdx.x * 256u + threadIdx.x; i < n; i += gridDim.x * 256u) {
        const float4 hr = P.ws.hitRec[i];
        if (q3_shades(__float_as_uint(P.ws.q3.rayD[i].w), __float_as_uint(hr.y))) continue;
        PathCtx c = path_ctx(P, nullptr, nullptr, nullptr);
        PathVars v;
        uint32_t p = 0, s = 0;
        HitInfo h;
        reload_entry(c, P.ws.q3, sc, i, hr, P.ws.hitErr[i], v, p, s, h);
        apply_hit(P, v.rs, h);
        if (!(v.rs.hitLight || !v.rs.isDiffuse || v.rs.isOccluded)) atomicAdd(&P.ws.counters[kCntError], 1u);
        store_path_L(c, v, p, s);
    }
}

constexpr int kChainRanges = 32;
#ifndef RTX_CHAIN_STATIC
#define RTX_CHAIN_STATIC 0
#endif
constexpr bool kChainStaticFirst = RTX_CHAIN_STATIC != 0;

template <bool kStats>
RT_DEV bool chain_step(const SceneView& sc, const TravRay& r, TravState& s, TravRec& rec, uint2* stk) {
    return trav_step<16, false, kStats>(sc, r, s, rec, stk, 256, nullptr);
}

#ifndef RTX_CHAIN_WAVES
#define RTX_CHAIN_WAVES 3
#endif
template <bool kStats>
__global__ __launch_bounds__(256, RTX_CHAIN_WAVES) void k_pt_chain(PathTraceParams P) {
    __shared__ uint2 stk[17 * 256];
    __shared__ uint32_t sob[256];
    __shared__ uint2 ranges[4][kChainRanges];
    __shared__ uint32_t q4list[4][64];
    __shared__ unsigned long long wgRays[4];
    const int tid = threadIdx.x, lane = tid & 63, w = __builtin_amdgcn_readfirstlane(tid >> 6);
    bn_stage_sobol(P.bluenoise, sob, tid, 256);
    __syncthreads();
    const uint32_t n = P.ws.counters[kCntQ3];
    const SceneView sc = scene_of(P);
    const PtQueue& q = P.ws.q3;
    const uint32_t allParts = (1u << kParts) - 1u;
    Fetch f;
    fetch_init(f, n, gridDim.x * 4u, blockIdx.x * 4u + (uint32_t)w, kChainStaticFirst);
    uint32_t rays = 0, rsD = 0;
#pragma unroll 1
    while (true) {
        uint32_t nRanges = 0;
        if (f.resLo < f.resHi) {
            if (lane == 0) ranges[w][0] = make_uint2(f.resLo, f.resHi);
            nRanges = 1;
        }
        bool active = false, exhausted = false, occlusion = false;
        uint32_t idx = 0;
        TravRay r;
        TravState s;
        TravRec rec;
// ... 2 lines not shown
#pragma unroll 1
        while (true) {
            const unsigned long long need = __ballot(!active && !exhausted);
            const unsigned long long busy = __ballot(active);
            if (need != 0ull && (__popcll(need) >= kRefillMin || busy == 0ull)) {
                const uint32_t k = (uint32_t)__popcll(need);
                if (f.resLo == f.resHi && nRanges < (uint32_t)kChainRanges) {
                    fetch_topup(f, n, P.ws.fetch, lane);
                    if (f.resLo < f.resHi) {
                        if (lane == 0) ranges[w][nRanges] = make_uint2(f.resLo, f.resHi);
                        ++nRanges;
                    }
                }
                const uint32_t avail = f.resHi - f.resLo;
                const bool none = avail == 0u;
                if (!active && !exhausted) {
                    const uint32_t rank = lane_rank(need);
                    if (rank < avail) {
                        idx = f.resLo + rank;
                        const float4 o = q.rayO[idx], d = q.rayD[idx];
                        trav_setup(sc, f3(o.x, o.y, o.z), f3(d.x, d.y, d.z), r);
                        trav_init(s, sc.root);
                        active = true;
                        occlusion = (__float_as_uint(d.w) & kQShadowFlag) != 0u;
                    } else if (none) {
                        exhausted = true;
                    }
                }
                f.resLo += k < avail ? k : avail;
            }
            if (__ballot(active) == 0ull) break;
            const bool tail = f.resLo == f.resHi && (f.drained == allParts || nRanges >= (uint32_t)kChainRanges);
            if (tail ? active : trav_lane_steps(active, s)) {
                bool done = false;
                do {
                    done = chain_step<kStats>(sc, r, s, rec, stk + tid) || s.iters >= 1024u || (occlusion && s.hitIdx >= 0);
                } while (tail && !done);
                if (done) {
                    P.ws.hitRec[idx] = make_float4(s.t, __uint_as_float((uint32_t)s.hitIdx), s.hitU, s.hitV);
                    P.ws.hitErr[idx] = s.hitErrT;
                    if (P.statsOut) {
                        const uint32_t p = __float_as_uint(q.rayO[idx].w);
                        atomicAdd(&P.statsOut[p].y, s.visits);
                        atomicAdd(&P.statsOut[p].z, s.tests);
                        atomicMax(&P.ws.counters[kCntMaxIter3], s.iters);
                        atomicAdd(&P.ws.counters[kCntVisQ3], s.visits);
                        atomicAdd(&P.ws.counters[kCntTstQ3], s.tests);
                    }
                    active = false;
                }
            }
        }
        __builtin_amdgcn_fence(__ATOMIC_SEQ_CST, "workgroup");
        PathCtx c = path_ctx(P, sob, P.skyTree, P.sunTree);
        uint32_t ri = 0, nq4 = 0;
#pragma unroll 1
        while (true) {
            const bool more = ri < nRanges;
            const uint2 rg = more ? ranges[w][ri] : make_uint2(0u, 0u);
            if (nq4 > 0u && (!more || nq4 + (rg.y - rg.x) > 64u)) {
                __builtin_amdgcn_fence(__ATOMIC_SEQ_CST, "workgroup");
                bool act = (uint32_t)lane < nq4;
                const uint32_t slot = act ? q4list[w][lane] : 0u;
                TravRay r4;
                TravState s4;
                {
                    const float4 o = P.ws.q4.rayO[slot], d = P.ws.q4.rayD[slot];
                    trav_setup(sc, f3(o.x, o.y, o.z), f3(d.x, d.y, d.z), r4);
                }
                trav_init(s4, sc.root);
                TravRec rec4;
                const bool mine = act;
                if (nq4 < 16u) {
#pragma unroll 1
                    while (act)
                        if (chain_step<kStats>(sc, r4, s4, rec4, stk + tid) || s4.iters >= 1024u || s4.hitIdx >= 0) act = false;
                } else {
#pragma unroll 1
                    while (__ballot(act) != 0ull) {
                        if (trav_lane_steps(act, s4)) {
                            if (chain_step<kStats>(sc, r4, s4, rec4, stk + tid) || s4.iters >= 1024u || s4.hitIdx >= 0)
                                act = false;
                        }
                    }
                }
                if (mine) {
                    PathVars v;
                    uint32_t p = 0, smp = 0;
                    c.rays = 0;
                    (void)resume_entry<4, false, false>(c, P.ws.q4, sc, slot,
                                                 make_float4(s4.t, __uint_as_float((uint32_t)s4.hitIdx), s4.hitU, s4.hitV),
                                                 s4.hitErrT, v, p, smp);
                    store_path_L(c, v, p, smp);
                    if (P.statsOut) {
                        atomicAdd(&P.statsOut[p].y, s4.visits);
                        atomicAdd(&P.statsOut[p].z, s4.tests);
                        atomicMax(&P.ws.counters[kCntMaxIter4], s4.iters);
                        atomicAdd(&P.ws.counters[kCntVisQ4], s4.visits);
                        atomicAdd(&P.ws.counters[kCntTstQ4], s4.tests);
                    }
                }
                nq4 = 0u;
                continue;
            }
            if (!more) break;
            const uint32_t i = rg.x + (uint32_t)lane;
            const bool act = i < rg.y;
// ... 215 lines not shown
```

### real-time-ray-tracing_amd/csrc/pt_common.h

```cpp
#pragma once
#include "bvh_kernels.h"
#include "rt_device.h"

namespace rtd {

constexpr float kPiOver4 = 0.7853981633974483096156608458198757210492f;
constexpr float kPiOver2 = 1.5707963267948966192313216916397514420985f;
constexpr float kPi = 3.1415926535897932384626422832795028841971f;
constexpr float kTwoPi = 6.2831853071795864769252867665590057683943f;

RT_DEV float div_by_const(float x, float d, float c) {
    const float q = x * c;
    const float fast = __builtin_fmaf(__builtin_fmaf(-q, d, x), c, q);
    const float ax = __builtin_fabsf(x);
    return (ax >= 0x1p-100f && ax <= 0x1.fffffep127f) ? fast : x / d;
}
RT_DEV float div_pi(float x) { return div_by_const(x, kPi, 0x1.45f306p-2f); }
RT_DEV float div_two_pi(float x) { return div_by_const(x, kTwoPi, 0x1.45f306p-3f); }

RT_DEV float bluenoise(const uint8_t* tables, int px, int py, int sampleIdx, int dim) {
    const uint8_t* sobol = tables;
    const uint8_t* scr = tables + 256 * 256;
    const uint8_t* rnk = scr + 128 * 128 * 8;
    px &= 127;
    py &= 127;
    sampleIdx &= 255;
    const int cell = (px + py * 128) * 8;
    const int ranked = sampleIdx ^ (int)rnk[dim + cell];
    int value = sobol[dim + ranked * 256];
    value = value ^ (int)scr[(dim % 8) + cell];
    return ((float)value + 0.5f) / 256.0f;
}

struct BnPixel {
    uint32_t rnk, scr;
};

RT_DEV BnPixel bn_pixel(const uint8_t* tables, int px, int py) {
    const uint8_t* scr = tables + 256 * 256;
    const uint8_t* rnk = scr + 128 * 128 * 8;
    const int cell = ((px & 127) + (py & 127) * 128) * 8;
    return BnPixel{*(const uint32_t*)(rnk + cell), *(const uint32_t*)(scr + cell)};
}

RT_DEV float bn_value(const uint32_t* sobolRows, BnPixel b, int sampleIdx, int dim) {
    const int sh = 8 * dim;
    const int ranked = (sampleIdx & 255) ^ (int)((b.rnk >> sh) & 255u);
    const int value = (int)((sobolRows[ranked] >> sh) & 255u) ^ (int)((b.scr >> sh) & 255u);
    return ((float)value + 0.5f) / 256.0f;
}

RT_DEV void bn_stage_sobol(const uint8_t* tables, uint32_t* sobolRows, int tid, int nthreads) {
    for (int r = tid; r < 256; r += nthreads) sobolRows[r] = *(const uint32_t*)(tables + r * 256);
}

RT_DEV F2 concentric_disk(F2 u) {
    const F2 o = {2.0f * u.x - 1.0f, 2.0f * u.y - 1.0f};
    if (fabsf(o.x) < 1e-10f && fabsf(o.y) < 1e-10f) return F2{0.0f, 0.0f};
    const bool xMajor = fabsf(o.x) > fabsf(o.y);
    const float r = xMajor ? o.x : o.y;
    const float q = (xMajor ? o.y : o.x) / r;
    const float theta = xMajor ? kPiOver4 * q : kPiOver2 - kPiOver4 * q;
    float sn, cs;
    rt_sincosf(theta, &sn, &cs);
    return F2{cs * r, sn * r};
}

RT_DEV F3 load3(const float* a) { return f3(a[0], a[1], a[2]); }

RT_DEV F3 center_dir(const TraceCamera& c, int ix, int iy) {
    F2 uvc = {((float)ix + 0.5f) * c.invRes[0], ((float)iy + 0.5f) * c.invRes[1]};
    uvc = F2{uvc.x * -2.0f + 1.0f, uvc.y * -2.0f + 1.0f};
    const F3 pc = load3(c.adjustedFront) + load3(c.adjustedLeft) * uvc.x + load3(c.adjustedUp) * uvc.y;
    return normalize(pc);
}

RT_DEV void generate_ray_jittered(const TraceCamera& c, int ix, int iy, F2 pix, F2 ap, F3& orig, F3& dir,
                                  F2& sampleUv) {
    F2 uv = {((float)ix + pix.x) * c.invRes[0], ((float)iy + pix.y) * c.invRes[1]};
    sampleUv = uv;
    uv = F2{uv.x * -2.0f + 1.0f, uv.y * -2.0f + 1.0f};
    const F3 p = load3(c.adjustedFront) + load3(c.adjustedLeft) * uv.x + load3(c.adjustedUp) * uv.y;
    const F2 d = concentric_disk(ap);
    const F3 pa = d.x * load3(c.apertureLeft) + d.y * load3(c.apertureUp);
    orig = load3(c.pos) + pa;
    dir = normalize(p - pa);
}

RT_DEV void generate_ray(const TraceCamera& c, int ix, int iy, F2 pix, F2 ap, F3& orig, F3& dir, F3& centerDir,
                         F2& sampleUv) {
    F2 uv = {((float)ix + pix.x) * c.invRes[0], ((float)iy + pix.y) * c.invRes[1]};
    F2 uvc = {((float)ix + 0.5f) * c.invRes[0], ((float)iy + 0.5f) * c.invRes[1]};
    sampleUv = uv;
    uv = F2{uv.x * -2.0f + 1.0f, uv.y * -2.0f + 1.0f};
    uvc = F2{uvc.x * -2.0f + 1.0f, uvc.y * -2.0f + 1.0f};
    const F3 front = load3(c.adjustedFront), left = load3(c.adjustedLeft), up = load3(c.adjustedUp);
    const F3 p = front + left * uv.x + up * uv.y;
    const F3 pc = front + left * uvc.x + up * uvc.y;
    const F2 d = concentric_disk(ap);
    const F3 pa = d.x * load3(c.apertureLeft) + d.y * load3(c.apertureUp);
    orig = load3(c.pos) + pa;
    dir = normalize(p - pa);
    centerDir = normalize(pc);
}

}
```

### real-time-ray-tracing_amd/csrc/shade.h

```cpp
#pragma once
#include "frame_kernels.h"
#include "pt_common.h"
#include "rtmath.h"

namespace rtd {

enum MatType : int { LAMBERTIAN = 0, PERFECT_REFLECTION = 1, FRESNEL_RR = 2, MICROFACET = 3, EMISSIVE = 4, MAT_SKY = 5 };
constexpr int kEnvLightId = 9999, kDefaultLightId = 7777;
constexpr float kInvTwoPi = 0.15915494309f;
constexpr float kSafeCos = 1e-5f;

RT_DEV int mat_type(int id) {
    switch (id) {
        case 0: case 2: return EMISSIVE;
        case 1: return FRESNEL_RR;
        case 3: case 6: case 7: case 8: case 9: return LAMBERTIAN;
        case 4: return MICROFACET;
        default: return PERFECT_REFLECTION;
    }
}
RT_DEV F3 mat_F0(int) { return f3(0.56f, 0.57f, 0.58f); }
RT_DEV float mat_alpha(int) { return 0.05f; }

RT_DEV F3 f3_4(float4 a) { return f3(a.x, a.y, a.z); }
// ... 101 lines not shown
    F3 o = f3(0.0f);
    float sw = 0.0f;
#pragma unroll
    for (int i = 0; i < 4; ++i) {
        sw += wt[i];
        int x = sx[i], y = sy[i];
        F3 c;
        if (kSun) {
            if (x < 0) x = 0;
            if (y < 0) y = 0;
            c = (x >= kSunW || y >= kSunH) ? f3(0.0f) : f3_4(buf[y * kSunW + x]);
        } else {
            if (x >= kSkyW) x %= kSkyW;
            if (x < 0) x = kSkyW - (-x) % kSkyW;
            if (x >= kSkyW) x = kSkyW - 1;
            if (y >= kSkyH) y = kSkyH - 1;
            if (y < 0) y = 0;
            c = f3_4(buf[y * kSkyW + x]);
        }
        o = o + c * wt[i];
    }
    return o / sw;
}

RT_DEV F3 env_light(const PathTraceParams& P, F3 sunDir, F3 rd) {
    F3 color;
    {
        const F2 uv = {div_two_pi(rt_atan2f(-rd.z, -rd.x)) + 0.5f, fmx(rd.y, 0.05f)};
        const F3 sky = bicubic_env<false>(P.skyBuffer, uv);
        const F3 mist = f3(0.2f);
        const float w = clampf((rd.y + 0.4f) * (1.0f / 0.5f));
        color = f3(0.0f) + (mist + (w * w * (3.0f - 2.0f * w)) * (sky - mist));
    }
    const float cosMax = P.cosThetaMax;
    const float cosTheta = inner3(sunDir.x, rd.x, sunDir.y, rd.y, sunDir.z, rd.z);
    if (cosTheta < cosMax) return color;
    const F3 c = f3(inner3(P.sunT[0], rd.x, P.sunT[1], rd.y, P.sunT[2], rd.z), cosTheta, 0.0f);
    const float u = (1.0f - cosTheta) / P.oneMinusCosThetaMax;
    const float sinTheta = __builtin_sqrtf(1.0f - cosTheta * cosTheta);
    if (sinTheta < 1e-5f || (c.x / sinTheta) < -1.0f || (c.x / sinTheta) > 1.0f) return color;
    const float v = rt_acosf(c.x / sinTheta) * kInvTwoPi;
    return color + bicubic_env<true>(P.sunBuffer, F2{u, v});
}

RT_DEV int cdf_search(const float* a, int left, int right, float target) {
    while (right - left > 1) {
        const int mid = (left + right) / 2;
        if (a[mid] < target) left = mid;
        else right = mid;
    }
    return left;
}

RT_DEV int cdf_search_tree(const float* a, int right, float target, const float* tree, int nodes) {
    int left = 0, j = 1;
    while (right - left > 1) {
        const int mid = (left + right) / 2;
        const float v = j < nodes ? tree[j] : a[mid];
        if (v < target) {
            left = mid;
            j = 2 * j + 1;
        } else {
            right = mid;
            j = 2 * j;
        }
    }
    return left;
}

RT_DEV void sample_light(const PathTraceParams& P, F3 sunDir, F3& dir, float& pdf, int& lightIdx, float r0, float r1,
                         const float* skyTree, const float* sunTree) {
    const float pSky = P.lightSel[0], maxSky = P.lightSel[1], maxSun = P.lightSel[2], sunDen = P.lightSel[3];
    if (pSky > r1) {
        const int idx = cdf_search_tree(P.skyCdf, kSkySize - 2, r0 * maxSky, skyTree, kSkyTreeNodes) + 1;
        float p = (P.skyCdf[idx] - P.skyCdf[idx - 1]) / maxSky;
        p = div_two_pi(p * kSkySize);
        const float u = ((float)(idx % kSkyW) + 0.5f) / kSkyW;
        const float v = ((float)(idx / kSkyW) + 0.5f) / kSkyH;
        dir = equal_area_map(u, v);
        pdf = p * 1.0f * pSky;
    } else {
        const int idx = cdf_search_tree(P.sunCdf, kSunSize - 2, r0 * maxSun, sunTree, kSunTreeNodes) + 1;
        float p = (P.sunCdf[idx] - P.sunCdf[idx - 1]) / maxSun;
        p = p * kSunSize / sunDen;
        const float u = ((float)(idx % kSunW) + 0.5f) / kSunW;
        const float v = ((float)(idx / kSunW) + 0.5f) / kSunH;
        dir = equal_area_map_cone(sunDir, f3(P.sunT[0], P.sunT[1], P.sunT[2]), f3(P.sunB[0], P.sunB[1], P.sunB[2]), u,
                                  v, P.cosThetaMax);
        pdf = p * 1.0f;
    }
    lightIdx = kEnvLightId;
}

RT_DEV void lambertian_sample(F2 u, F3& wo, F3 n) {
    const float r = __builtin_sqrtf(u.x);
    const float theta = kTwoPi * u.y;
    const F2 d = {r * rt_cosf(theta), r * rt_sinf(theta)};
    const float z = __builtin_sqrtf(max1f(0.0f, 1.0f - d.x * d.x - d.y * d.y));
    F3 uu, vv;
    localize_sample(n, uu, vv);
    wo = normalize(d.x * uu + d.y * vv + z * n);
}

RT_DEV F3 fresnel_schlick(F3 F0, float cosTheta) {
    const float e = 1.0f - cosTheta;
    const float e2 = e * e;
    return F0 + (f3(1.0f) - F0) * (e2 * e2 * e);
}

RT_DEV void microfacet_terms(F3 wo, F3 wi, F3 wh, F3 wn, F3 F0, F3 albedo, float alpha2, F3& brdfOverPdf, F3& brdf,
                             float& pdf) {
    const float cWoWh = fmx(kSafeCos, dot(wh, wo));
    const F3 F = fresnel_schlick(F0, cWoWh);
    const float cWo = clampf(dot(wo, wn), kSafeCos, 1.0f - kSafeCos);
    const float cWi = fmx(kSafeCos, dot(wi, wn));
    const float tWo = __builtin_sqrtf(1.0f - cWo * cWo) / cWo;
    const float G = 1.0f / (1.0f + (__builtin_sqrtf(1.0f + alpha2 * tWo * tWo) - 1.0f) / 2.0f);
    const float cWh = fmx(kSafeCos, dot(wh, wn));
    const float c2 = cWh * cWh;
    const float t2 = (1.0f - c2) / c2;
    const float e = t2 / alpha2 + 1.0f;
    const float D = 1.0f / (kPi * (alpha2 * c2 * c2) * (e * e));
    brdf = (albedo * F) * (D * G) / (4.0f * cWo * cWi);
    pdf = (D * cWh) / (4.0f * cWoWh);
    brdfOverPdf = (albedo * F) * (G * cWoWh) / (cWh * cWo);
}

RT_DEV F3 reflect3(F3 i, F3 n) { return i - 2.0f * n * dot(n, i); }

RT_DEV F3 ggx_normal(F2 r, float alpha2, F3 normal) {
    const float cosTheta = 1.0f / __builtin_sqrtf(1.0f + alpha2 * r.x / (1.0f - r.x));
    const float sinTheta = __builtin_sqrtf(1.0f - cosTheta * cosTheta);
    const float phi = kTwoPi * r.y;
    const F3 sl = f3(sinTheta * rt_cosf(phi), cosTheta, sinTheta * rt_sinf(phi));
    F3 t, b;
    localize_sample(normal, t, b);
    return normalize(sl.x * t + sl.z * b + sl.y * normal);
}

}
```

### real-time-ray-tracing_amd/csrc/sky.hip

```cpp
#include "frame_kernels.h"
#include "rt_device.h"
#include "rtmath.h"
#include "shade.h"

using namespace rtd;

namespace {

RT_DEV F3 xyz_to_srgb(F3 c) {
    const float m00 = (float)3.2404542, m01 = (float)-1.5371385, m02 = (float)-0.4985314;
    const float m10 = (float)-0.9692660, m11 = (float)1.8760108, m12 = (float)0.0415560;
    const float m20 = (float)0.0556434, m21 = (float)-0.2040259, m22 = (float)1.0572252;
    return f3(inner3(m00, c.x, m01, c.y, m02, c.z), inner3(m10, c.x, m11, c.y, m12, c.z),
              inner3(m20, c.x, m21, c.y, m22, c.z));
}

RT_DEV F3 sky_radiance(F3 rd, F3 sunDir, const SkyGenParams& P) {
    const float theta = rt_acosf(rd.y);
    const float gamma = rt_acosf(clampf(dot(rd, sunDir), -1.0f, 1.0f));
    const float cg = rt_cosf(gamma), ct = rt_cosf(theta);
    const float zenith = __builtin_sqrtf(ct);
    F3 xyz = f3(0.0f);
    for (int ch = 0; ch < 10; ++ch) {
        const float* c = P.st.configs + ch * 9;
// ... 86 lines not shown
    if (t == 0) {
        if (sums) sums[blockIdx.x] = a[n - 1];
        a[n - 1] = 0.0f;
    }
    for (int d = 1; d < n; d *= 2) {
        offset >>= 1;
        __syncthreads();
        for (int i = t; i < d; i += T) {
            const int ai = offset * (2 * i + 1) - 1, bi = offset * (2 * i + 2) - 1;
            const float tmp = a[ai];
            a[ai] = a[bi];
            a[bi] = a[bi] + tmp;
        }
    }
    __syncthreads();
    float* dst = out + (size_t)blockIdx.x * n;
    for (int i = t; i < n; i += T) dst[i] = kInclusive ? a[i] + src[i] : a[i];
}

__global__ __launch_bounds__(256) void k_scan_add(float* out, const float* sums, int n, int total) {
    const int i = blockIdx.x * 256 + threadIdx.x;
    if (i < total) out[i] = out[i] + sums[i / n];
}

extern "C" hipError_t rtk_launch_scan_ex(const float* in, float* out, float* sums, int size, int blockSize,
                                         int postfix, hipStream_t stream) {
    if (blockSize < 2 || blockSize > 8192 || (blockSize & (blockSize - 1)) || size < blockSize || size % blockSize)
        return hipErrorInvalidValue;
    const int blocks = size / blockSize;
    if (blocks > 8192 || (blocks & (blocks - 1)) || (blocks > 1 && !sums)) return hipErrorInvalidValue;
    const int thr = blockSize / 2 < 256 ? blockSize / 2 : 256;
    const size_t lds = (size_t)blockSize * sizeof(float);
    if (postfix)
        hipLaunchKernelGGL(k_scan_block<true>, dim3(blocks), dim3(thr), lds, stream, in, out, blocks > 1 ? sums : nullptr,
                           blockSize);
    else
        hipLaunchKernelGGL(k_scan_block<false>, dim3(blocks), dim3(thr), lds, stream, in, out,
                           blocks > 1 ? sums : nullptr, blockSize);
    if (blocks > 1) {
        const int st = blocks / 2 < 256 ? blocks / 2 : 256;
        hipLaunchKernelGGL(k_scan_block<false>, dim3(1), dim3(st), (size_t)blocks * sizeof(float), stream,
                           (const float*)sums, sums, (float*)nullptr, blocks);
        hipLaunchKernelGGL(k_scan_add, dim3((size + 255) / 256), dim3(256), 0, stream, out, (const float*)sums,
                           blockSize, size);
    }
    return hipGetLastError();
}

extern "C" hipError_t rtk_launch_scan(const float* in, float* out, float* sums, int size, int blockSize,
                                      hipStream_t stream) {
    return rtk_launch_scan_ex(in, out, sums, size, blockSize, 1, stream);
}

__global__ void k_cdf_tree(const float* cdf, int right0, float* tree, int nodes) {
    const int j = blockIdx.x * blockDim.x + threadIdx.x;
    if (j >= nodes) return;
    if (j == 0) { tree[0] = __builtin_nanf(""); return; }
    const int depth = 31 - __clz(j);
    int left = 0, right = right0;
    bool live = right - left > 1;
    for (int b = depth - 1; b >= 0 && live; --b) {
        const int mid = (left + right) / 2;
        if ((j >> b) & 1) left = mid;
        else right = mid;
        live = right - left > 1;
    }
    tree[j] = live ? cdf[(left + right) / 2] : __builtin_nanf("");
}

__global__ void k_light_select(const float* skyCdf, const float* sunCdf, float cosThetaMax, float* out) {
    const float maxSky = skyCdf[kSkySize - 1], maxSun = sunCdf[kSunSize - 1];
    const float totalSky = maxSky * kTwoPi / kSkySize;
    const float totalSun = maxSun * kTwoPi * (1.0f - cosThetaMax) / kSunSize;
    out[0] = totalSky / (totalSky + totalSun);
    out[1] = maxSky;
    out[2] = maxSun;
    out[3] = kTwoPi * (1.0f - cosThetaMax);
}

extern "C" hipError_t rtk_launch_sky(const SkyGenParams* p, hipStream_t stream) {
    hipLaunchKernelGGL(k_sky, dim3(kSkySize / 256), dim3(256), 0, stream, *p);
    hipError_t e = rtk_launch_scan(p->skyPdf, p->skyCdf, p->scanSums, kSkySize, kSkyScanBlock, stream);
    if (e != hipSuccess) return e;
    hipLaunchKernelGGL(k_sun, dim3(kSunSize / 256), dim3(256), 0, stream, *p);
    if ((e = rtk_launch_scan(p->sunPdf, p->sunCdf, p->scanSums, kSunSize, kSunScanBlock, stream)) != hipSuccess)
        return e;
    hipLaunchKernelGGL(k_cdf_tree, dim3(kSkyTreeNodes / 256), dim3(256), 0, stream, p->skyCdf, kSkySize - 2,
                       p->skyTree, kSkyTreeNodes);
    hipLaunchKernelGGL(k_cdf_tree, dim3(kSunTreeNodes / 256), dim3(256), 0, stream, p->sunCdf, kSunSize - 2,
                       p->sunTree, kSunTreeNodes);
    hipLaunchKernelGGL(k_light_select, dim3(1), dim3(1), 0, stream, (const float*)p->skyCdf, (const float*)p->sunCdf,
                       p->cosThetaMax, p->lightSel);
    return hipGetLastError();
}
```

### real-time-ray-tracing_amd/csrc/trace_primary.hip

```cpp
#include "bvh_kernels.h"
#include "pt_common.h"
#include "traverse.h"

using namespace rtd;

template <bool kStats>
#ifndef RTX_PRIMARY_WPE
__global__ __launch_bounds__(256) void k_trace_primary(TracePrimaryParams P) {
#else
__global__ __launch_bounds__(256) __attribute__((amdgpu_waves_per_eu(RTX_PRIMARY_WPE, RTX_PRIMARY_WPE)))
void k_trace_primary(TracePrimaryParams P) {
#endif
    constexpr int kLds = 10;
    __shared__ uint2 stk[kLds * 256];
    const int tid = threadIdx.x, lane = tid & 63, w = tid >> 6;
    const int x = blockIdx.x * 16 + (w & 1) * 8 + (lane & 7);
    const int yl = blockIdx.y * 16 + (w >> 1) * 8 + (lane >> 3);
    if (x >= (int)P.width || yl >= (int)P.rows) return;
    const int y = (int)row_of(P.y0, P.nStrips, P.strip, (uint32_t)yl);

    const int s = P.frameNum * 4 + 0;
    const F2 pix = {bluenoise(P.bluenoise, x, y, s, 0), bluenoise(P.bluenoise, x, y, s, 1)};
    const F2 ap = {bluenoise(P.bluenoise, x, y, s, 2), bluenoise(P.bluenoise, x, y, s, 3)};
    F3 org, dir, centerDir;
    F2 sampleUv;
    generate_ray(P.cam, x, y, pix, ap, org, dir, centerDir, sampleUv);

    const SceneView sc = scene_view(P.nodes, P.tlasNodes, P.triPos, P.triNrm);
    HitInfo hi;
    intersect<kLds, kStats>(sc, org, dir, stk + tid, 256, hi);

    const size_t p = (size_t)y * P.width + x;
    P.hitOut[p] = make_float4(hi.t, __int_as_float(hi.objectIdx), hi.u, hi.v);
    if (P.normalOut) P.normalOut[p] = make_float4(hi.normal.x, hi.normal.y, hi.normal.z, hi.hit ? 1.0f : 0.0f);
    if (P.fakeNormalOut) P.fakeNormalOut[p] = make_float4(hi.fakeNormal.x, hi.fakeNormal.y, hi.fakeNormal.z, hi.offset);
    if (kStats) {
        P.statsOut[4 * p + 0] = hi.visits;
        P.statsOut[4 * p + 1] = hi.tests;
        P.statsOut[4 * p + 2] = hi.dropped;
        P.statsOut[4 * p + 3] = hi.iters;
    }
}

extern "C" hipError_t rtk_launch_trace_primary(const TracePrimaryParams* p, hipStream_t stream) {
    dim3 grid((p->width + 15) / 16, (p->rows + 15) / 16);
    if (p->statsOut) hipLaunchKernelGGL(k_trace_primary<true>, grid, dim3(256), 0, stream, *p);
    else hipLaunchKernelGGL(k_trace_primary<false>, grid, dim3(256), 0, stream, *p);
    return hipGetLastError();
}

__global__ __launch_bounds__(256) void k_smooth_normals(const float* V, const uint32_t* adjOffsets,
                                                        const uint32_t* adjCorners, const uint32_t* indices,
                                                        uint32_t nverts, float* N) {
    const uint32_t vtx = blockIdx.x * 256 + threadIdx.x;
    if (vtx >= nverts) return;
    F3 acc = f3(0.0f);
    const uint32_t a0 = adjOffsets[vtx], a1 = adjOffsets[vtx + 1];
    for (int pass = 0; pass < 2; ++pass) {
        for (uint32_t a = a0; a < a1; ++a) {
            const uint32_t c = adjCorners[a];
            const uint32_t t = c / 3, k = c - 3 * t;
            const uint32_t i0 = indices[3 * t], i1 = indices[3 * t + 1], i2 = indices[3 * t + 2];
            const F3 v0 = f3(V[3 * i0], V[3 * i0 + 1], V[3 * i0 + 2]);
            const F3 v1 = f3(V[3 * i1], V[3 * i1 + 1], V[3 * i1 + 2]);
            const F3 v2 = f3(V[3 * i2], V[3 * i2 + 1], V[3 * i2 + 2]);
            const F3 pnma = cross(v2 - v0, v2 - v1) / 2.0f;
            F3 ea, eb;
            if (k == 0) { ea = v2 - v0; eb = v1 - v0; }
            else if (k == 1) { ea = v2 - v1; eb = v0 - v1; }
            else { ea = v0 - v2; eb = v1 - v2; }
            const float wgt = rt_acosf(dot(ea, eb) / __builtin_sqrtf(length2(ea) * length2(eb)));
            acc = acc + pnma * wgt;
        }
    }
    N[3 * vtx] = acc.x;
    N[3 * vtx + 1] = acc.y;
    N[3 * vtx + 2] = acc.z;
}

// ... 8 lines not shown
```

### real-time-ray-tracing_amd/rtx/__init__.py

```python
from __future__ import annotations

import ctypes as C
import os

import numpy as np

_PKG = os.path.dirname(os.path.dirname(os.path.abspath(__file__)))
LIB_PATH = os.path.join(_PKG, "lib", "librtx.so")
DATA_DIR = os.path.join(_PKG, "data")

RT_OK = 0
ERRORS = {-1: "RT_ERR_ARG", -2: "RT_ERR_HIP", -3: "RT_ERR_IO", -4: "RT_ERR_STATE", -5: "RT_ERR_NO_DEVICE", -6: "RT_ERR_DEVICE"}

ARR = dict(VERTICES=0, INDICES=1, NORMALS=2, TRI_POS=3, AABBS=4, MORTON=5, REORDER=6, NODES=7, TLAS_AABBS=8,
           TLAS_MORTON=9, TLAS_REORDER=10, TLAS_NODES=11, TLAS_SCENE_AABB=12, BATCH_SCENE_AABBS=13, HITS=14,
           HIT_NORMALS=15, HIT_FAKE_NORMALS=16, HIT_STATS=17, TRI_NRM=18, RAYS=19, SKY_PDF=20, SKY_CDF=21,
           SUN_PDF=22, SUN_CDF=23, SUN_DIR=24, HISTOGRAM=25, EXPOSURE=26, COLOR4=27, COLOR16=28, COLOR64=29,
           RGBA8=30, PT_STATS=31, PT_QUEUE=32, PT_Q3_ORIGINS=33, PT_Q3_DIRS=34,
           PT_Q4_ORIGINS=35, PT_Q4_DIRS=36, TEX_ALBEDO_AO=37, TEX_NORMAL_ROUGHNESS=38, TEX_HEIGHT=39, HDR=40,
           BVH_ARENA=41, TRI_MATERIALS=42, ADJ_OFFSETS=43, CORNER_SLOTS=44, TRI_MATERIAL_CENSUS=45)
TEX = dict(SOIL_ALBEDO_AO=0, SOIL_NORMAL_ROUGHNESS=1, SOIL_HEIGHT=2)
BUF = dict(RENDER_COLOR=0, ACCUMULATION=1, HISTORY_COLOR=2, SCALED_COLOR=3, NORMAL=10, DEPTH=11, HISTORY_DEPTH=12,
           MOTION=13, NOISE_LEVEL=14, NOISE_LEVEL16=15, SKY=16, SUN=17, ALBEDO=18, RGBA8=19, HISTOGRAM=20)

# ... 82 lines not shown

    __hash__ = None

    def __repr__(self):
        return "Material(type=%d, flags=%d, color=%s, emission=%s, ior=%r, alpha=%r, f0=%s)" % (
            self.type, self.flags, list(self.color), list(self.emission), self.ior, self.alpha, list(self.f0))


MAT_LAMBERTIAN, MAT_MIRROR, MAT_GLASS, MAT_MICROFACET, MAT_EMISSIVE = range(5)
MAT_FLAG_FLAT = 1

QUERY_ANY_HIT = 1
QUERY_MAX_RAYS = 1 << 30

COLLECTIVE_FN = C.CFUNCTYPE(C.c_int, C.c_void_p, C.c_int, C.c_void_p, C.POINTER(StripExchange))
HOOK_HISTOGRAM, HOOK_ROWS, HOOK_GBUFFERS = 0, 1, 2


SIGNATURES = {
    "rt_create": (C.c_int, [C.c_int, C.c_int, C.c_char_p, C.POINTER(C.c_void_p)]),
    "rt_init": (C.c_int, [C.c_void_p]),
    "rt_draw": (C.c_int, [C.c_void_p, C.c_void_p, C.c_void_p]),
    "rt_draw_device": (C.c_int, [C.c_void_p, C.c_void_p, C.c_size_t, C.c_int]),
    "rt_destroy": (None, [C.c_void_p]),
    "rt_last_error": (C.c_char_p, [C.c_void_p]),
    "rt_get_params": (C.c_int, [C.c_void_p, C.POINTER(Params)]),
    "rt_set_params": (C.c_int, [C.c_void_p, C.POINTER(Params)]),
    "rt_get_camera": (C.c_int, [C.c_void_p, C.POINTER(Camera)]),
    "rt_set_camera": (C.c_int, [C.c_void_p, C.POINTER(Camera)]),
    "rt_set_frame_index": (C.c_int, [C.c_void_p, C.c_int]),
    "rt_set_delta_time": (C.c_int, [C.c_void_p, C.c_float]),
    "rt_keyboard_update": (C.c_int, [C.c_void_p, C.c_int, C.c_int, C.c_int, C.c_int]),
    "rt_cursor_pos_update": (C.c_int, [C.c_void_p, C.c_double, C.c_double]),
    "rt_scroll_update": (C.c_int, [C.c_void_p, C.c_double, C.c_double]),
    "rt_mouse_button_update": (C.c_int, [C.c_void_p, C.c_int, C.c_int, C.c_int]),
    "rt_set_cursor_reset": (C.c_int, [C.c_void_p, C.c_int]),
    "rt_get_info": (C.c_int, [C.c_void_p, C.POINTER(Info)]),
    "rt_get_buffer": (C.c_int, [C.c_void_p, C.c_int, C.c_void_p, C.c_size_t]),
    "rt_buffer_bytes": (C.c_size_t, [C.c_void_p, C.c_int]),
    "rt_path_trace": (C.c_int, [C.c_void_p, C.c_int, C.c_int]),
    "rt_denoise_post": (C.c_int, [C.c_void_p, C.c_int, C.c_int]),
    "rt_set_stream": (C.c_int, [C.c_void_p, C.c_void_p]),
    "rt_set_post_stream": (C.c_int, [C.c_void_p, C.c_void_p]),
    "rt_set_gather_stream": (C.c_int, [C.c_void_p, C.c_void_p]),
    "rt_bind_buffer": (C.c_int, [C.c_void_p, C.c_int, C.c_void_p, C.c_size_t]),
    "rt_set_collective_hook": (C.c_int, [C.c_void_p, C.c_void_p, C.c_void_p]),
    "rt_set_hook_stages": (C.c_int, [C.c_void_p, C.c_uint32]),
    "rt_get_ray_count": (C.c_int, [C.c_void_p, C.POINTER(C.c_uint64), C.c_int]),
    "rt_build_bvh": (C.c_int, [C.c_void_p]),
    "rt_trace_primary": (C.c_int, [C.c_void_p, C.c_int, C.c_int]),
    "rt_sync": (C.c_int, [C.c_void_p]),
    "rt_time_stage": (C.c_int, [C.c_void_p, C.c_int, C.c_int, C.POINTER(C.c_float)]),
    "rt_debug_pk_math": (C.c_int, [C.c_int, C.c_void_p, C.c_float, C.c_float, C.c_void_p, C.c_void_p, C.c_size_t]),
    "rt_time_path_trace_kernels": (C.c_int, [C.c_void_p, C.c_int, C.POINTER(C.c_float), C.c_int]),
    "rt_time_frame_kernels": (C.c_int, [C.c_void_p, C.c_int, C.c_int, C.POINTER(C.c_float), C.c_int]),
    "rt_trace_rays": (C.c_int, [C.c_void_p, C.c_void_p, C.c_uint32, C.c_void_p, C.c_void_p, C.POINTER(C.c_float)]),
    "rt_trace_rays_device": (C.c_int, [C.c_void_p, C.POINTER(RayQuery)]),
    "rt_download": (C.c_int, [C.c_void_p, C.c_int, C.c_void_p, C.c_size_t]),
    "rt_array_bytes": (C.c_size_t, [C.c_void_p, C.c_int]),
    "rt_save_camera": (C.c_int, [C.c_void_p, C.c_char_p]),
    "rt_load_camera": (C.c_int, [C.c_void_p, C.c_char_p]),
    "rt_save_image": (C.c_int, [C.c_void_p, C.c_char_p, C.c_int]),
    "rt_upload_texture": (C.c_int, [C.c_void_p, C.c_int, C.c_void_p, C.c_int, C.c_int, C.c_int]),
    "rt_scene_noise3d": (C.c_int, [C.c_void_p, C.c_size_t, C.c_void_p]),
    "rt_filter_kernel": (C.c_int, [C.c_int, C.c_void_p, C.c_int]),
    "rt_scan_device": (C.c_int, [C.c_void_p, C.c_void_p, C.c_void_p, C.c_int, C.c_int, C.c_int, C.c_void_p]),
    "rt_frame_marks_begin": (C.c_int, [C.c_void_p, C.c_int, C.c_uint32]),
    "rt_frame_marks_read": (C.c_int, [C.c_void_p, C.POINTER(C.c_float), C.c_int, C.POINTER(C.c_int)]),
    "rt_update_vertices": (C.c_int, [C.c_void_p, C.c_void_p, C.c_uint32, C.c_uint32]),
    "rt_update_vertices_device": (C.c_int, [C.c_void_p, C.c_void_p, C.c_uint32, C.c_uint32, C.c_void_p]),
    "rt_get_geometry_epoch": (C.c_int, [C.c_void_p, C.POINTER(C.c_uint64)]),
    "rt_set_mesh": (C.c_int, [C.c_void_p, C.POINTER(Mesh)]),
    "rt_set_mesh_device": (C.c_int, [C.c_void_p, C.POINTER(Mesh)]),
    "rt_mesh_adjacency": (C.c_int, [C.c_void_p, C.c_uint32, C.c_uint32, C.c_void_p, C.c_void_p, C.c_void_p]),
    "rt_time_mesh_set": (C.c_int, [C.c_void_p, C.c_int, C.POINTER(C.c_float)]),
    "rt_set_geometry_motion": (C.c_int, [C.c_void_p, C.c_int]),
    "rt_get_geometry_motion": (C.c_int, [C.c_void_p, C.POINTER(C.c_int)]),
    "rt_set_triangle_materials": (C.c_int, [C.c_void_p, C.c_void_p, C.c_uint32, C.c_uint32]),
    "rt_reset_triangle_materials": (C.c_int, [C.c_void_p]),
    "rt_material_classes": (C.c_int, [C.c_void_p, C.c_size_t, C.POINTER(C.c_uint32)]),
    "rt_set_triangle_materials_device": (C.c_int, [C.c_void_p, C.POINTER(MaterialUpdate)]),
    "rt_material_class_rule": (C.c_uint32, [C.c_uint32]),
    "rt_default_material": (C.c_int, [C.c_uint32, C.POINTER(Material)]),
    "rt_set_materials": (C.c_int, [C.c_void_p, C.c_uint32, C.c_uint32, C.POINTER(Material)]),
    "rt_get_materials": (C.c_int, [C.c_void_p, C.c_uint32, C.c_uint32, C.POINTER(Material)]),
    "rt_reset_materials": (C.c_int, [C.c_void_p]),
}
MAT_CLASS_GLOSSY, MAT_CLASS_MICROFACET = 1, 2
MAT_CLASS_ALL = MAT_CLASS_GLOSSY | MAT_CLASS_MICROFACET
IMAGE_PPM_RGBA8, IMAGE_PFM_HDR = 0, 1
DRAW_ASYNC = 1
BUF_SET1, BUF_SET2, BUF_SET3 = 0x100, 0x200, 0x300
GBUFFER_SETS = 4

_lib = None


def load_library(path: str | None = None) -> C.CDLL:
    global _lib
    if _lib is not None:
        return _lib
    path = path or os.environ.get("RTX_LIB") or LIB_PATH
    if not os.path.exists(path):
        raise RuntimeError("librtx.so not found at %s — run `make` (or __graft_entry__.build())" % path)
    try:
        import torch
# ... 335 lines not shown
    def frame_marks_read(self):
        ms = (C.c_float * len(self.FRAME_KERNELS))()
        n = C.c_int()
        self._check(self.lib.rt_frame_marks_read(self.h, ms, len(ms), C.byref(n)), "rt_frame_marks_read")
        return {k: float(v) for k, v in zip(self.FRAME_KERNELS, ms) if v >= 0.0}, n.value

    def save_camera(self, path: str):
        self._check(self.lib.rt_save_camera(self.h, path.encode()), "rt_save_camera")

    def load_camera(self, path: str):
        self._check(self.lib.rt_load_camera(self.h, path.encode()), "rt_load_camera")

    def save_image(self, path: str, kind: int = IMAGE_PPM_RGBA8):
        self._check(self.lib.rt_save_image(self.h, path.encode(), kind), "rt_save_image")

    def upload_texture(self, name: str, texels: np.ndarray):
        t = np.ascontiguousarray(texels, np.uint16)
        h, w = t.shape[:2]
        c = 1 if t.ndim == 2 else t.shape[2]
        self._check(self.lib.rt_upload_texture(self.h, TEX[name], t.ctypes.data, w, h, c), "rt_upload_texture")

    def download(self, name: str, dtype=np.uint8) -> np.ndarray:
        what = ARR[name]
        n = self.lib.rt_array_bytes(self.h, what)
        buf = np.empty(n, dtype=np.uint8)
        self._check(self.lib.rt_download(self.h, what, buf.ctypes.data, n), "rt_download(%s)" % name)
        return buf.view(dtype)

    def trace_rays(self, org, dirs, want_iters=False):
        org = np.asarray(org, np.float32).reshape(-1, 3)
        dirs = np.asarray(dirs, np.float32).reshape(-1, 3)
        n = len(org)
        rays = np.zeros((n, 8), np.float32)
        rays[:, 0:3] = org
        rays[:, 4:7] = dirs
        hits = np.zeros((n, 4), np.float32)
        iters = np.zeros(n, np.uint32) if want_iters else None
        ms = C.c_float()
        self._check(self.lib.rt_trace_rays(self.h, rays.ctypes.data, n, hits.ctypes.data, _ptr(iters), C.byref(ms)),
                    "rt_trace_rays")
        out = (hits[:, 0], hits[:, 1].view(np.int32), hits[:, 2], hits[:, 3])
        return out + ((iters,) if want_iters else ()) + (ms.value,)

    def trace_rays_device(self, org_ptr: int, dir_ptr: int, n: int, hits_ptr: int, *, org_stride: int = 3,
                          dir_stride: int = 3, iters_ptr: int | None = None, any_hit: bool = False,
                          ready_event: int | None = None, done_event: int | None = None):
        for name, v in (("n", n), ("org_stride", org_stride), ("dir_stride", dir_stride)):
            if not 0 <= int(v) <= 0xFFFFFFFF:
                raise ValueError("trace_rays_device: %s must fit 32 bits" % name)
        q = RayQuery(org_ptr, int(org_stride), dir_ptr, int(dir_stride), int(n), hits_ptr, iters_ptr,
                     QUERY_ANY_HIT if any_hit else 0, ready_event, done_event)
        self._check(self.lib.rt_trace_rays_device(self.h, C.byref(q)), "rt_trace_rays_device")

    def get_buffer(self, name: str, shape=None, dtype=np.uint8) -> np.ndarray:
        if shape is None:
            n = self.lib.rt_buffer_bytes(self.h, BUF[name])
            shape = (n // np.dtype(dtype).itemsize,)
        out = np.empty(shape, dtype=dtype)
        self._check(self.lib.rt_get_buffer(self.h, BUF[name], out.ctypes.data, out.nbytes), "rt_get_buffer")
        return out


def material_classes(ids) -> int:
    a = np.ascontiguousarray(ids, dtype=np.uint8).reshape(-1)
    c = C.c_uint32()
    rc = load_library().rt_material_classes(a.ctypes.data if a.size else None, a.size, C.byref(c))
    if rc != RT_OK:
        raise RtError("rt_material_classes: %s" % ERRORS.get(rc, rc))
    return c.value


def default_material(id: int) -> Material:
    if not 0 <= int(id) <= 0xFFFFFFFF:
        raise ValueError("default_material: id must fit 32 bits")
    m = Material()
    rc = load_library().rt_default_material(int(id), C.byref(m))
    if rc != RT_OK:
        raise RtError("rt_default_material: %s" % ERRORS.get(rc, rc))
    return m


def mesh_adjacency(indices_padded, nv: int):
    a = np.ascontiguousarray(indices_padded, dtype=np.uint32).reshape(-1)
    if a.size % 3:
        raise ValueError("mesh_adjacency: three indices per triangle")
    off = np.empty(int(nv) + 1, np.uint32)
    corners = np.empty(a.size, np.uint32)
    slots = np.empty(a.size, np.uint32)
    rc = load_library().rt_mesh_adjacency(a.ctypes.data, a.size // 3, int(nv), off.ctypes.data, corners.ctypes.data,
                                          slots.ctypes.data)
    if rc != RT_OK:
        raise RtError("rt_mesh_adjacency: %s" % ERRORS.get(rc, rc))
    return off, corners, slots


def _ptr(a):
    if a is None:
        return None
    assert a.flags["C_CONTIGUOUS"]
    return a.ctypes.data
```

Baseline: 11880 Mray/s.

## Precompute blue-noise-indexed lookup tables for light, lambertian, GGX and lens sampling

Blue-noise samples are quantized to 256 byte values, so the sampling functions that consume them can be precomputed into tables. Light sampling directions and pdfs, cos/sin of 2πu, sqrt(u) and the concentric lens disk are built once per sky update or at init. The path tracer stages these tables in LDS and does indexed lookups in place of CDF tree searches and transcendental math. This removes per-bounce binary searches and trig from the hot shading loop, at the cost of LDS footprint, which may lower occupancy, and extra table-build kernels. A debug entry point compares the stored tables against direct evaluation.

```diff
diff --git a/include/rtx_amd.h b/include/rtx_amd.h
--- a/include/rtx_amd.h
+++ b/include/rtx_amd.h
@@ -251,6 +251,8 @@
 int rt_time_mesh_set(rt_context* ctx, int iters, float* parts_ms);
 
 int rt_debug_pk_math(int fn, const float* x, float y, float c, float* out_pk, float* out_scalar, size_t n);
+
+int rt_debug_rng_tables(rt_context* ctx, int which, void* stored, void* direct, size_t bytes);
 
 int rt_time_path_trace_kernels(rt_context* ctx, int iters, float* kernel_ms, int n);
 
diff --git a/real-time-ray-tracing_amd/csrc/bvh_kernels.h b/real-time-ray-tracing_amd/csrc/bvh_kernels.h
--- a/real-time-ray-tracing_amd/csrc/bvh_kernels.h
+++ b/real-time-ray-tracing_amd/csrc/bvh_kernels.h
@@ -1,6 +1,13 @@
 #pragma once
 #include <hip/hip_runtime.h>
 #include <stdint.h>
+
+#ifndef RTX_RNG_TABLES
+#define RTX_RNG_TABLES 1
+#endif
+#ifndef RTX_RNG_LENS_CAMERA
+#define RTX_RNG_LENS_CAMERA 0
+#endif
 
 constexpr int kStatusTlasTimeout = 0;
 constexpr int kStatusTlasTimeoutBuild = 1;
@@ -83,6 +90,7 @@
     uint32_t nStrips, strip;
     int frameNum;
     const uint8_t* bluenoise;
+    const float2* lensDisk;
     const float4* triPos;
     const float4* triNrm;
     const void* nodes;
diff --git a/real-time-ray-tracing_amd/csrc/context.cpp b/real-time-ray-tracing_amd/csrc/context.cpp
--- a/real-time-ray-tracing_amd/csrc/context.cpp
+++ b/real-time-ray-tracing_amd/csrc/context.cpp
@@ -1207,6 +1207,7 @@
     p.strip = (uint32_t)ctx->stripIndex;
     p.frameNum = frame_num;
     p.bluenoise = ctx->dBlueNoise;
+    p.lensDisk = ctx->fr.lensDisk;
     p.triPos = ctx->dTriPos;
     p.triNrm = ctx->dTriNrm;
     p.nodes = ctx->dNodes;
diff --git a/real-time-ray-tracing_amd/csrc/context.h b/real-time-ray-tracing_amd/csrc/context.h
--- a/real-time-ray-tracing_amd/csrc/context.h
+++ b/real-time-ray-tracing_amd/csrc/context.h
@@ -58,8 +58,14 @@
     float* sunPdf = nullptr;
     float* sunCdf = nullptr;
     float* scanSums = nullptr;
+#if !RTX_RNG_TABLES
     float* skyTree = nullptr;
     float* sunTree = nullptr;
+#endif
+    float2* lensDisk = nullptr;
+    float2* unitTrig = nullptr;
+    float* unitSqrt = nullptr;
+    float4* lightTab = nullptr;
     float* lightSel = nullptr;
     bool skyValid = false;
     rt_sky_params lastSky{};
diff --git a/real-time-ray-tracing_amd/csrc/debug_math.hip b/real-time-ray-tracing_amd/csrc/debug_math.hip
--- a/real-time-ray-tracing_amd/csrc/debug_math.hip
+++ b/real-time-ray-tracing_amd/csrc/debug_math.hip
@@ -1,7 +1,9 @@
 #include <hip/hip_runtime.h>
 
+#include "frame_kernels.h"
 #include "rtmath_pk.h"
 #include "rtx_amd.h"
+#include "shade.h"
 
 namespace {
 __global__ __launch_bounds__(256) void k_debug_pk(int fn, const float* x, float y, float c, float* outPk,
@@ -24,6 +26,45 @@
     outPk[i] = pk;
     outScalar[i] = sc;
 }
+
+__global__ __launch_bounds__(256) void k_debug_rng_direct(PathTraceParams P, int which, void* out) {
+    using namespace rtd;
+    const int i = (int)(blockIdx.x * 256u + threadIdx.x);
+    if (which == 0) {
+        if (i >= 256 * 256) return;
+        const F2 d = concentric_disk(F2{bn_float(i >> 8), bn_float(i & 255)});
+        static_cast<float2*>(out)[i] = make_float2(d.x, d.y);
+    } else if (which == 1) {
+        if (i >= 256) return;
+        const float theta = kTwoPi * bn_float(i);
+        static_cast<float2*>(out)[i] = make_float2(rt_cosf(theta), rt_sinf(theta));
+    } else if (which == 2) {
+        if (i >= 256) return;
+        static_cast<float*>(out)[i] = __builtin_sqrtf(bn_float(i));
+    } else {
+        if (i >= kLightTabSize) return;
+        LightFrame L{};
+        L.skyCdf = P.skyCdf;
+        L.sunCdf = P.sunCdf;
+        L.lightSel = P.lightSel;
+        L.sunDir = f3(P.sunDir[0], P.sunDir[1], P.sunDir[2]);
+        L.sunT = f3(P.sunT[0], P.sunT[1], P.sunT[2]);
+        L.sunB = f3(P.sunB[0], P.sunB[1], P.sunB[2]);
+        L.cosThetaMax = P.cosThetaMax;
+        F3 dir;
+        float pdf;
+        int lightIdx;
+        sample_light(L, dir, pdf, lightIdx, bn_float(i >> 1), bn_float((i & 1) ? 255 : 0));
+        static_cast<float4*>(out)[i] = make_float4(dir.x, dir.y, dir.z, pdf);
+    }
+}
+}
+
+extern "C" hipError_t rtk_debug_rng_direct(const PathTraceParams* p, int which, void* direct, hipStream_t stream) {
+    if (which < 0 || which > 3 || !direct) return hipErrorInvalidValue;
+    const unsigned n = which == 0 ? 256u * 256u : which == 3 ? (unsigned)rtd::kLightTabSize : 256u;
+    hipLaunchKernelGGL(k_debug_rng_direct, dim3((n + 255u) / 256u), dim3(256), 0, stream, *p, which, direct);
+    return hipGetLastError();
 }
 
 extern "C" int rt_debug_pk_math(int fn, const float* x, float y, float c, float* out_pk, float* out_scalar, size_t n) {
diff --git a/real-time-ray-tracing_amd/csrc/frame.cpp b/real-time-ray-tracing_amd/csrc/frame.cpp
--- a/real-time-ray-tracing_amd/csrc/frame.cpp
+++ b/real-time-ray-tracing_amd/csrc/frame.cpp
@@ -93,6 +93,8 @@
     return true;
 }
 
+void sun_frame(const float n[3], float t[3], float b[3]);
+
 bool sky_params_equal(const rt_sky_params& a, const rt_sky_params& b) {
     return a.timeOfDay == b.timeOfDay && a.sunAxisAngle == b.sunAxisAngle && a.skyScalar == b.skyScalar &&
            a.sunScalar == b.sunScalar && a.sunAngle == b.sunAngle;
@@ -135,9 +137,13 @@
     p.sunPdf = fr.sunPdf;
     p.sunCdf = fr.sunCdf;
     p.scanSums = fr.scanSums;
+#if !RTX_RNG_TABLES
     p.skyTree = fr.skyTree;
     p.sunTree = fr.sunTree;
+#endif
     p.lightSel = fr.lightSel;
+    sun_frame(fr.sunDir, p.sunT, p.sunB);
+    p.lightTab = fr.lightTab;
     HIP_TRY(ctx, rtk_launch_sky(&p, ctx->stream));
     if (ctx->postStream) HIP_TRY(ctx, hipStreamSynchronize(ctx->stream));
     fr.sunArea = rt_powf(rt_tanf(sunRadius), 2.0f) * kPi;
@@ -396,9 +402,17 @@
     ALLOC(fr.sunPdf, (size_t)kSunSize * 4);
     ALLOC(fr.sunCdf, (size_t)kSunSize * 4);
     ALLOC(fr.scanSums, 512 * 4);
+#if !RTX_RNG_TABLES
     ALLOC(fr.skyTree, (size_t)kSkyTreeNodes * 4);
     ALLOC(fr.sunTree, (size_t)kSunTreeNodes * 4);
+#endif
     ALLOC(fr.lightSel, 16);
+    ALLOC(fr.lensDisk, (size_t)256 * 256 * 8);
+    ALLOC(fr.unitTrig, 256 * 8);
+    ALLOC(fr.unitSqrt, 256 * 4);
+    ALLOC(fr.lightTab, (size_t)512 * 16);
+    HIP_TRY(ctx, rtk_launch_rng_tables(fr.lensDisk, fr.unitTrig, fr.unitSqrt, ctx->stream));
+    HIP_TRY(ctx, hipStreamSynchronize(ctx->stream));
     ALLOC(fr.texAlbedo, (size_t)kTexTexels * 8);
     ALLOC(fr.texNormal, (size_t)kTexTexels * 8);
     ALLOC(fr.texHeight, (size_t)kTexTexels * 2);
@@ -631,9 +645,15 @@
     p.sunBuffer = fr.sun;
     p.skyCdf = fr.skyCdf;
     p.sunCdf = fr.sunCdf;
+#if !RTX_RNG_TABLES
     p.skyTree = fr.skyTree;
     p.sunTree = fr.sunTree;
+#endif
     p.lightSel = fr.lightSel;
+    p.lensDisk = fr.lensDisk;
+    p.unitTrig = fr.unitTrig;
+    p.unitSqrt = fr.unitSqrt;
+    p.lightTab = fr.lightTab;
     memcpy(p.sunDir, fr.sunDir, 12);
     p.cosThetaMax = fr.cosThetaMax;
     p.oneMinusCosThetaMax = 1.0f - fr.cosThetaMax;
@@ -1578,3 +1598,32 @@
     if (q->done_event) HIP_TRY(ctx, hipEventRecord((hipEvent_t)q->done_event, s));
     return RT_OK;
 }
+
+int rt_debug_rng_tables(rt_context* ctx, int which, void* stored, void* direct, size_t bytes) {
+    if (!ctx || !stored || !direct || which < 0 || which > 4) return RT_ERR_ARG;
+    if (!ctx->inited) { ctx->err = "rt_debug_rng_tables before rt_init"; return RT_ERR_STATE; }
+    FrameResources& fr = ctx->fr;
+    const size_t need = which == 0 ? (size_t)256 * 256 * 8 : which == 1 ? 256 * 8 : which == 2 ? 256 * 4 : which == 3 ? 512 * 16 : 16;
+    if (bytes < need) { ctx->err = "destination too small"; return RT_ERR_ARG; }
+    if (int rc = update_sky(ctx)) return rc;
+    if (int rc = sync_streams(ctx)) return rc;
+    const void* table = which == 0 ? (const void*)fr.lensDisk : which == 1 ? (const void*)fr.unitTrig
+                      : which == 2 ? (const void*)fr.unitSqrt : which == 3 ? (const void*)fr.lightTab : (const void*)fr.lightSel;
+    HIP_TRY(ctx, hipMemcpy(stored, table, need, hipMemcpyDeviceToHost));
+    if (which == 4) {
+        memcpy(direct, stored, need);
+        return RT_OK;
+    }
+    HostCamera hc;
+    rt_camera_update(ctx->camera, ctx->renderW, ctx->renderH, hc);
+    PathTraceParams p;
+    (void)fill_pt_params(ctx, 1, 0, hc, fr.gbSet, p);
+    void* d = nullptr;
+    HIP_TRY(ctx, hipMalloc(&d, need));
+    hipError_t e = rtk_debug_rng_direct(&p, which, d, ctx->stream);
+    if (e == hipSuccess) e = hipStreamSynchronize(ctx->stream);
+    if (e == hipSuccess) e = hipMemcpy(direct, d, need, hipMemcpyDeviceToHost);
+    (void)hipFree(d);
+    HIP_TRY(ctx, e);
+    return RT_OK;
+}
diff --git a/real-time-ray-tracing_amd/csrc/frame_kernels.h b/real-time-ray-tracing_amd/csrc/frame_kernels.h
--- a/real-time-ray-tracing_amd/csrc/frame_kernels.h
+++ b/real-time-ray-tracing_amd/csrc/frame_kernels.h
@@ -36,12 +36,18 @@
     float* sunPdf;
     float* sunCdf;
     float* scanSums;
+#if !RTX_RNG_TABLES
     float* skyTree;
     float* sunTree;
+#endif
     float* lightSel;
-};
-
+    float sunT[3], sunB[3];
+    float4* lightTab;
+};
+
+#if !RTX_RNG_TABLES
 constexpr int kSkyTreeNodes = 4096, kSunTreeNodes = 1024;
+#endif
 
 struct HistCamera { float pos[3], left[3], up[3], dir[3]; };
 
@@ -133,8 +139,14 @@
     const float4* sunBuffer;
     const float* skyCdf;
     const float* sunCdf;
+#if !RTX_RNG_TABLES
     const float* skyTree;
     const float* sunTree;
+#endif
+    const float2* lensDisk;
+    const float2* unitTrig;
+    const float* unitSqrt;
+    const float4* lightTab;
     const float* lightSel;
     float sunDir[3];
     float sunT[3], sunB[3];
@@ -238,6 +250,8 @@
 extern "C" hipError_t rtk_hdr_out(const uint2* color, float4* hdr, size_t n, hipStream_t stream);
 
 extern "C" hipError_t rtk_launch_sky(const SkyGenParams* p, hipStream_t stream);
+extern "C" hipError_t rtk_launch_rng_tables(float2* lensDisk, float2* unitTrig, float* unitSqrt, hipStream_t stream);
+extern "C" hipError_t rtk_debug_rng_direct(const PathTraceParams* p, int which, void* direct, hipStream_t stream);
 extern "C" hipError_t rtk_launch_mipgen(uint16_t* chain, int size, int levels, int channels, hipStream_t stream);
 extern "C" hipError_t rtk_launch_scan(const float* in, float* out, float* sums, int size, int blockSize,
                                       hipStream_t stream);
diff --git a/real-time-ray-tracing_amd/csrc/pathtrace.hip b/real-time-ray-tracing_amd/csrc/pathtrace.hip
--- a/real-time-ray-tracing_amd/csrc/pathtrace.hip
+++ b/real-time-ray-tracing_amd/csrc/pathtrace.hip
@@ -18,6 +18,33 @@
     bool isRayIntoSurface, hitLight, hit, isDiffuse, isHitProcessed, isOccluded, isShadowRay;
     float offset, normalDotRayDir, depth, rayConeWidth, rayConeSpread;
 };
+
+struct ShadeTabs {
+#if RTX_RNG_TABLES
+    const float4* light = nullptr;
+    const float2* trig = nullptr;
+    const float* sqrt = nullptr;
+#else
+    const float* skyTree = nullptr;
+    const float* sunTree = nullptr;
+#endif
+};
+
+#if !RTX_RNG_TABLES
+RT_DEV LightFrame light_frame(const PathTraceParams& P, F3 sunDir, const ShadeTabs& t) {
+    LightFrame L{};
+    L.skyCdf = P.skyCdf;
+    L.sunCdf = P.sunCdf;
+    L.lightSel = P.lightSel;
+    L.sunDir = sunDir;
+    L.sunT = f3(P.sunT[0], P.sunT[1], P.sunT[2]);
+    L.sunB = f3(P.sunB[0], P.sunB[1], P.sunB[2]);
+    L.cosThetaMax = P.cosThetaMax;
+    L.skyTree = t.skyTree;
+    L.sunTree = t.sunTree;
+    return L;
+}
+#endif
 
 struct PathCtx {
     const PathTraceParams& P;
@@ -26,20 +53,52 @@
     BnPixel bp;
     int frameIdx;
     uint32_t rays, visits, tests, diffuse;
-    const float* skyTree = nullptr;
-    const float* sunTree = nullptr;
+    ShadeTabs tabs;
 };
 
-RT_DEV PathCtx path_ctx(const PathTraceParams& P, const uint32_t* sob, const float* skyTree, const float* sunTree) {
-    return PathCtx{P, f3(P.sunDir[0], P.sunDir[1], P.sunDir[2]), sob, BnPixel{0u, 0u}, 0, 0u, 0u, 0u, 0u, skyTree, sunTree};
-}
-
-RT_DEV void stage_cdf_trees(const PathTraceParams& P, float* sky, float* sun, int tid, int nthreads) {
-    for (int i = tid; i < kSkyTreeNodes / 4; i += nthreads) reinterpret_cast<float4*>(sky)[i] = reinterpret_cast<const float4*>(P.skyTree)[i];
-    for (int i = tid; i < kSunTreeNodes / 4; i += nthreads) reinterpret_cast<float4*>(sun)[i] = reinterpret_cast<const float4*>(P.sunTree)[i];
-}
-
-RT_DEV float rnd(const PathCtx& c, int k, int d) { return bn_value(c.sob, c.bp, c.frameIdx * 4 + k, d); }
+RT_DEV PathCtx path_ctx(const PathTraceParams& P, const uint32_t* sob, ShadeTabs tabs = ShadeTabs{}) {
+    return PathCtx{P, f3(P.sunDir[0], P.sunDir[1], P.sunDir[2]), sob, BnPixel{0u, 0u}, 0, 0u, 0u, 0u, 0u, tabs};
+}
+
+RT_DEV ShadeTabs global_tabs(const PathTraceParams& P) {
+#if RTX_RNG_TABLES
+    return ShadeTabs{P.lightTab, P.unitTrig, P.unitSqrt};
+#else
+    return ShadeTabs{P.skyTree, P.sunTree};
+#endif
+}
+
+template <bool kOn>
+struct ShadeLds {};
+template <>
+struct alignas(16) ShadeLds<true> {
+#if RTX_RNG_TABLES
+    float4 light[kLightTabSize];
+    float2 trig[256];
+    float sqrt[256];
+#else
+    float sky[kSkyTreeNodes];
+    float sun[kSunTreeNodes];
+#endif
+};
+RT_DEV ShadeTabs stage_shade_tabs(const PathTraceParams& P, ShadeLds<true>& l, int tid, int nthreads) {
+#if RTX_RNG_TABLES
+    for (int i = tid; i < kLightTabSize; i += nthreads) l.light[i] = P.lightTab[i];
+    for (int i = tid; i < 256; i += nthreads) {
+        l.trig[i] = P.unitTrig[i];
+        l.sqrt[i] = P.unitSqrt[i];
+    }
+    return ShadeTabs{l.light, l.trig, l.sqrt};
+#else
+    for (int i = tid; i < kSkyTreeNodes / 4; i += nthreads) reinterpret_cast<float4*>(l.sky)[i] = reinterpret_cast<const float4*>(P.skyTree)[i];
+    for (int i = tid; i < kSunTreeNodes / 4; i += nthreads) reinterpret_cast<float4*>(l.sun)[i] = reinterpret_cast<const float4*>(P.sunTree)[i];
+    return ShadeTabs{l.sky, l.sun};
+#endif
+}
+RT_DEV ShadeTabs stage_shade_tabs(const PathTraceParams&, ShadeLds<false>&, int, int) { return ShadeTabs{}; }
+
+RT_DEV int rnd_byte(const PathCtx& c, int k, int d) { return bn_byte(c.sob, c.bp, c.frameIdx * 4 + k, d); }
+RT_DEV float rnd(const PathCtx& c, int k, int d) { return bn_float(rnd_byte(c, k, d)); }
 
 struct PathVars {
     RayState rs;
@@ -182,21 +241,34 @@
         albedo = flat ? f3(m0.x, m0.y, m0.z) : albedo * f3(m0.x, m0.y, m0.z);
     }
     if (bounce == 0) rs.albedo = albedo * (1.0f + fabsf(dot(normal, rs.centerRaydir)));
-    float r[4], r2[4];
+    int rb[4];
 #pragma unroll
-    for (int d = 0; d < 4; ++d) {
-        r[d] = rnd(c, 2 * bounce, d);
-        r2[d] = rnd(c, 2 * bounce + 1, d);
-    }
+    for (int d = 0; d < 4; ++d) rb[d] = rnd_byte(c, 2 * bounce, d);
+    const int lb0 = rnd_byte(c, 2 * bounce + 1, 0);
+    const float l1 = rnd(c, 2 * bounce + 1, 1);
     const F3 rayDir = rs.dir;
     F3 lDir;
     float lPdf = 1.0f;
     int lIdx;
-    sample_light(P, c.sunDir, lDir, lPdf, lIdx, r2[0], r2[1], c.skyTree, c.sunTree);
+#if RTX_RNG_TABLES
+    sample_light_table(c.tabs.light, P.lightSel, lDir, lPdf, lIdx, lb0, l1);
+    auto ggx = [&](int i, int j, float alpha2) {
+        const float2 t = c.tabs.trig[rb[j]];
+        return ggx_normal_dir(bn_float(rb[i]), t.x, t.y, alpha2, normal);
+    };
+#else
+    sample_light<true>(light_frame(P, c.sunDir, c.tabs), lDir, lPdf, lIdx, bn_float(lb0), l1);
+    auto ggx = [&](int i, int j, float alpha2) { return ggx_normal(F2{bn_float(rb[i]), bn_float(rb[j])}, alpha2, normal); };
+#endif
     F3 sDir, sBsdf, lBsdf, tmp;
     float sPdf = 0.0f;
     if (!kMF || rs.matType == LAMBERTIAN) {
-        lambertian_sample(F2{r[0], r[1]}, sDir, normal);
+#if RTX_RNG_TABLES
+        const float2 t = c.tabs.trig[rb[1]];
+        lambertian_dir(c.tabs.sqrt[rb[0]], t.x, t.y, sDir, normal);
+#else
+        lambertian_sample(F2{bn_float(rb[0]), bn_float(rb[1])}, sDir, normal);
+#endif
         sBsdf = f3(div_pi(albedo.x), div_pi(albedo.y), div_pi(albedo.z));
         sPdf = div_pi(fmx(dot(sDir, normal), kSafeCos));
         lBsdf = sBsdf;
@@ -209,10 +281,10 @@
             alpha = m1.w;
         }
         const float alpha2 = alpha * alpha;
-        const F3 sn = ggx_normal(F2{r[0], r[1]}, alpha2, normal);
+        const F3 sn = ggx(0, 1, alpha2);
         sDir = normalize(reflect3(rayDir, sn));
         if (dot(sDir, surfaceNormal) < 0.0f) {
-            const F3 sn2 = ggx_normal(F2{r[2], r[3]}, alpha2, normal);
+            const F3 sn2 = ggx(2, 3, alpha2);
             sDir = normalize(reflect3(rayDir, sn2));
             if (dot(sDir, surfaceNormal) < 0.0f) sDir = normalize(reflect3(rayDir, normal));
         }
@@ -226,7 +298,7 @@
     if (lPdf != lPdf) lPdf = 0.0f;
     const float ph = (sPdf * sPdf) / (sPdf * sPdf + lPdf * lPdf);
     const float minPdf = 1e-5f;
-    if (r[3] < ph) {
+    if (bn_float(rb[3]) < ph) {
         if (dot(rs.normal, sDir) < 0.0f) { rs.isOccluded = true; return; }
         const float cwi = fmx(kSafeCos, dot(sDir, normal));
         beta = sBsdf * cwi / fmx(sPdf, minPdf);
@@ -414,8 +486,9 @@
     rs.rayConeWidth = 0.0f;
     rs.rayConeSpread = coneSpread;
     rs.centerRaydir = centerDir;
-    generate_ray_jittered(c.P.cam, x, y, F2{rnd(c, 0, 0), rnd(c, 0, 1)}, F2{rnd(c, 0, 2), rnd(c, 0, 3)}, rs.orig,
-                          rs.dir, v.sampleUv);
+    generate_ray_jittered(c.P.cam, x, y, F2{rnd(c, 0, 0), rnd(c, 0, 1)},
+                          lens_disk<kRngTables>(c.P.lensDisk, rnd_byte(c, 0, 2), rnd_byte(c, 0, 3)), rs.orig, rs.dir,
+                          v.sampleUv);
     v.outDepth = 0.0f;
     v.mask = 0u;
     v.mv = F2{0.0f, 0.0f};
@@ -449,7 +522,7 @@
     const uint32_t pl = (uint32_t)yl * P.width + (uint32_t)x;
     const size_t plane = (size_t)P.rows * P.width;
     const SceneView sc = scene_of(P);
-    PathCtx c = path_ctx(P, sob, nullptr, nullptr);
+    PathCtx c = path_ctx(P, sob);
     if (active) c.bp = bn_pixel(P.bluenoise, x, y);
     const int rounds = kOneRound ? 1 : ((int)P.spp + nSW - 1) / nSW;
     F3 L = f3(0.0f), A = f3(0.0f);
@@ -465,8 +538,9 @@
             c.frameIdx = (int)P.spp * (P.frameNum - 1) + 1 + s;
             F3 org, dir;
             F2 uv;
-            generate_ray_jittered(P.cam, x, y, F2{rnd(c, 0, 0), rnd(c, 0, 1)}, F2{rnd(c, 0, 2), rnd(c, 0, 3)}, org,
-                                  dir, uv);
+            generate_ray_jittered(P.cam, x, y, F2{rnd(c, 0, 0), rnd(c, 0, 1)},
+                                  lens_disk<kRngLensCamera>(P.lensDisk, rnd_byte(c, 0, 2), rnd_byte(c, 0, 3)), org, dir,
+                                  uv);
             TravState st;
             if (root_surely_missed(sc, org, dir)) {
                 trav_root_miss(st, sc.root);
@@ -615,13 +689,12 @@
     __shared__ float4 foldL[4][64];
     __shared__ float4 foldA[4][64];
     __shared__ unsigned long long wgRays[4];
-    __shared__ __align__(16) float sSkyTree[kSkyTreeNodes];
-    __shared__ __align__(16) float sSunTree[kSunTreeNodes];
+    __shared__ ShadeLds<true> sTabs;
     __shared__ uint32_t wgBatch;
     const int tid = threadIdx.x, lane = tid & 63, w = tid >> 6;
     const int wS = __builtin_amdgcn_readfirstlane(w);
     bn_stage_sobol(P.bluenoise, sob, tid, 256);
-    stage_cdf_trees(P, sSkyTree, sSunTree, tid, 256);
+    const ShadeTabs tabs = stage_shade_tabs(P, sTabs, tid, 256);
     __syncthreads();
     const uint32_t n = P.ws.counters[kCntSurface];
     const int nSW = cam_sample_waves(P.spp), sw = w % nSW, g = w / nSW;
@@ -640,7 +713,7 @@
         const int x = (int)(pl % P.width), yl = (int)(pl / P.width);
         const int y = (int)row_of(P.y0, P.nStrips, P.strip, (uint32_t)yl);
         const uint32_t p = (uint32_t)y * P.width + (uint32_t)x;
-        PathCtx c = path_ctx(P, sob, sSkyTree, sSunTree);
+        PathCtx c = path_ctx(P, sob, tabs);
         float coneSpread = 0.0f;
         F3 centerDir = f3(0.0f);
         if (active) {
@@ -783,7 +856,7 @@
         const int x = (int)(pl % P.width), yl = (int)(pl / P.width);
         const int y = (int)row_of(P.y0, P.nStrips, P.strip, (uint32_t)yl);
         const uint32_t p = (uint32_t)y * P.width + (uint32_t)x;
-        PathCtx c = path_ctx(P, sob, nullptr, nullptr);
+        PathCtx c = path_ctx(P, sob);
         c.bp = bn_pixel(P.bluenoise, x, y);
         c.frameIdx = (int)P.spp * (P.frameNum - 1) + 1;
         PathVars v;
@@ -886,13 +959,12 @@
     static_assert(!kListed || (kStep == 3 && !kGlossy), "the shading list is queue 3's, kept without glossy tables");
     __shared__ uint32_t sob[256];
     __shared__ unsigned long long wgRays[4];
-    __shared__ __align__(16) float sSkyTree[kStep == 3 ? kSkyTreeNodes : 4];
-    __shared__ __align__(16) float sSunTree[kStep == 3 ? kSunTreeNodes : 4];
+    __shared__ ShadeLds<kStep == 3> sTabs;
     const uint32_t n = P.ws.counters[kListed ? kCntShade3 : kStep == 3 ? kCntQ3 : kCntQ4];
     if (blockIdx.x * 256u >= n) return;
     const int tid = threadIdx.x;
     bn_stage_sobol(P.bluenoise, sob, tid, 256);
-    if (kStep == 3) stage_cdf_trees(P, sSkyTree, sSunTree, tid, 256);
+    const ShadeTabs tabs = stage_shade_tabs(P, sTabs, tid, 256);
     __syncthreads();
     const PtQueue& q = kStep == 3 ? P.ws.q3 : P.ws.q4;
     const float4* hitRec = kStep == 3 ? P.ws.hitRec : P.ws.hitRec4;
@@ -903,7 +975,7 @@
     for (uint32_t base = blockIdx.x * 256u; base < n; base += gridDim.x * 256u) {
         const uint32_t li = base + (uint32_t)tid;
         const bool active = li < n;
-        PathCtx c = path_ctx(P, sob, sSkyTree, sSunTree);
+        PathCtx c = path_ctx(P, sob, tabs);
         PathVars v;
         int kd = 5;
         uint32_t p = 0, s = 0;
@@ -935,7 +1007,7 @@
     for (uint32_t i = blockIdx.x * 256u + threadIdx.x; i < n; i += gridDim.x * 256u) {
         const float4 hr = P.ws.hitRec[i];
         if (q3_shades(__float_as_uint(P.ws.q3.rayD[i].w), __float_as_uint(hr.y))) continue;
-        PathCtx c = path_ctx(P, nullptr, nullptr, nullptr);
+        PathCtx c = path_ctx(P, nullptr);
         PathVars v;
         uint32_t p = 0, s = 0;
         HitInfo h;
@@ -1044,7 +1116,7 @@
             }
         }
         __builtin_amdgcn_fence(__ATOMIC_SEQ_CST, "workgroup");
-        PathCtx c = path_ctx(P, sob, P.skyTree, P.sunTree);
+        PathCtx c = path_ctx(P, sob, global_tabs(P));
         uint32_t ri = 0, nq4 = 0;
 #pragma unroll 1
         while (true) {
diff --git a/real-time-ray-tracing_amd/csrc/pt_common.h b/real-time-ray-tracing_amd/csrc/pt_common.h
--- a/real-time-ray-tracing_amd/csrc/pt_common.h
+++ b/real-time-ray-tracing_amd/csrc/pt_common.h
@@ -3,6 +3,9 @@
 #include "rt_device.h"
 
 namespace rtd {
+
+constexpr bool kRngTables = RTX_RNG_TABLES != 0;
+constexpr bool kRngLensCamera = kRngTables && RTX_RNG_LENS_CAMERA != 0;
 
 constexpr float kPiOver4 = 0.7853981633974483096156608458198757210492f;
 constexpr float kPiOver2 = 1.5707963267948966192313216916397514420985f;
@@ -18,7 +21,9 @@
 RT_DEV float div_pi(float x) { return div_by_const(x, kPi, 0x1.45f306p-2f); }
 RT_DEV float div_two_pi(float x) { return div_by_const(x, kTwoPi, 0x1.45f306p-3f); }
 
-RT_DEV float bluenoise(const uint8_t* tables, int px, int py, int sampleIdx, int dim) {
+RT_DEV float bn_float(int b) { return ((float)b + 0.5f) / 256.0f; }
+
+RT_DEV int bluenoise_byte(const uint8_t* tables, int px, int py, int sampleIdx, int dim) {
     const uint8_t* sobol = tables;
     const uint8_t* scr = tables + 256 * 256;
     const uint8_t* rnk = scr + 128 * 128 * 8;
@@ -29,7 +34,10 @@
     const int ranked = sampleIdx ^ (int)rnk[dim + cell];
     int value = sobol[dim + ranked * 256];
     value = value ^ (int)scr[(dim % 8) + cell];
-    return ((float)value + 0.5f) / 256.0f;
+    return value;
+}
+RT_DEV float bluenoise(const uint8_t* tables, int px, int py, int sampleIdx, int dim) {
+    return bn_float(bluenoise_byte(tables, px, py, sampleIdx, dim));
 }
 
 struct BnPixel {
@@ -43,11 +51,13 @@
     return BnPixel{*(const uint32_t*)(rnk + cell), *(const uint32_t*)(scr + cell)};
 }
 
-RT_DEV float bn_value(const uint32_t* sobolRows, BnPixel b, int sampleIdx, int dim) {
+RT_DEV int bn_byte(const uint32_t* sobolRows, BnPixel b, int sampleIdx, int dim) {
     const int sh = 8 * dim;
     const int ranked = (sampleIdx & 255) ^ (int)((b.rnk >> sh) & 255u);
-    const int value = (int)((sobolRows[ranked] >> sh) & 255u) ^ (int)((b.scr >> sh) & 255u);
-    return ((float)value + 0.5f) / 256.0f;
+    return (int)((sobolRows[ranked] >> sh) & 255u) ^ (int)((b.scr >> sh) & 255u);
+}
+RT_DEV float bn_value(const uint32_t* sobolRows, BnPixel b, int sampleIdx, int dim) {
+    return bn_float(bn_byte(sobolRows, b, sampleIdx, dim));
 }
 
 RT_DEV void bn_stage_sobol(const uint8_t* tables, uint32_t* sobolRows, int tid, int nthreads) {
@@ -66,6 +76,16 @@
     return F2{cs * r, sn * r};
 }
 
+template <bool kTable>
+RT_DEV F2 lens_disk(const float2* lensDisk, int b2, int b3) {
+    if constexpr (kTable) {
+        const float2 d = lensDisk[b2 * 256 + b3];
+        return F2{d.x, d.y};
+    } else {
+        return concentric_disk(F2{bn_float(b2), bn_float(b3)});
+    }
+}
+
 RT_DEV F3 load3(const float* a) { return f3(a[0], a[1], a[2]); }
 
 RT_DEV F3 center_dir(const TraceCamera& c, int ix, int iy) {
@@ -75,19 +95,18 @@
     return normalize(pc);
 }
 
-RT_DEV void generate_ray_jittered(const TraceCamera& c, int ix, int iy, F2 pix, F2 ap, F3& orig, F3& dir,
+RT_DEV void generate_ray_jittered(const TraceCamera& c, int ix, int iy, F2 pix, F2 d, F3& orig, F3& dir,
                                   F2& sampleUv) {
     F2 uv = {((float)ix + pix.x) * c.invRes[0], ((float)iy + pix.y) * c.invRes[1]};
     sampleUv = uv;
     uv = F2{uv.x * -2.0f + 1.0f, uv.y * -2.0f + 1.0f};
     const F3 p = load3(c.adjustedFront) + load3(c.adjustedLeft) * uv.x + load3(c.adjustedUp) * uv.y;
-    const F2 d = concentric_disk(ap);
     const F3 pa = d.x * load3(c.apertureLeft) + d.y * load3(c.apertureUp);
     orig = load3(c.pos) + pa;
     dir = normalize(p - pa);
 }
 
-RT_DEV void generate_ray(const TraceCamera& c, int ix, int iy, F2 pix, F2 ap, F3& orig, F3& dir, F3& centerDir,
+RT_DEV void generate_ray(const TraceCamera& c, int ix, int iy, F2 pix, F2 d, F3& orig, F3& dir, F3& centerDir,
                          F2& sampleUv) {
     F2 uv = {((float)ix + pix.x) * c.invRes[0], ((float)iy + pix.y) * c.invRes[1]};
     F2 uvc = {((float)ix + 0.5f) * c.invRes[0], ((float)iy + 0.5f) * c.invRes[1]};
@@ -97,7 +116,6 @@
     const F3 front = load3(c.adjustedFront), left = load3(c.adjustedLeft), up = load3(c.adjustedUp);
     const F3 p = front + left * uv.x + up * uv.y;
     const F3 pc = front + left * uvc.x + up * uvc.y;
-    const F2 d = concentric_disk(ap);
     const F3 pa = d.x * load3(c.apertureLeft) + d.y * load3(c.apertureUp);
     orig = load3(c.pos) + pa;
     dir = normalize(p - pa);
diff --git a/real-time-ray-tracing_amd/csrc/shade.h b/real-time-ray-tracing_amd/csrc/shade.h
--- a/real-time-ray-tracing_amd/csrc/shade.h
+++ b/real-time-ray-tracing_amd/csrc/shade.h
@@ -177,6 +177,7 @@
     return left;
 }
 
+#if !RTX_RNG_TABLES
 RT_DEV int cdf_search_tree(const float* a, int right, float target, const float* tree, int nodes) {
     int left = 0, j = 1;
     while (right - left > 1) {
@@ -192,39 +193,81 @@
     }
     return left;
 }
-
-RT_DEV void sample_light(const PathTraceParams& P, F3 sunDir, F3& dir, float& pdf, int& lightIdx, float r0, float r1,
-                         const float* skyTree, const float* sunTree) {
-    const float pSky = P.lightSel[0], maxSky = P.lightSel[1], maxSun = P.lightSel[2], sunDen = P.lightSel[3];
-    if (pSky > r1) {
-        const int idx = cdf_search_tree(P.skyCdf, kSkySize - 2, r0 * maxSky, skyTree, kSkyTreeNodes) + 1;
-        float p = (P.skyCdf[idx] - P.skyCdf[idx - 1]) / maxSky;
-        p = div_two_pi(p * kSkySize);
-        const float u = ((float)(idx % kSkyW) + 0.5f) / kSkyW;
-        const float v = ((float)(idx / kSkyW) + 0.5f) / kSkyH;
-        dir = equal_area_map(u, v);
-        pdf = p * 1.0f * pSky;
-    } else {
-        const int idx = cdf_search_tree(P.sunCdf, kSunSize - 2, r0 * maxSun, sunTree, kSunTreeNodes) + 1;
-        float p = (P.sunCdf[idx] - P.sunCdf[idx - 1]) / maxSun;
-        p = p * kSunSize / sunDen;
-        const float u = ((float)(idx % kSunW) + 0.5f) / kSunW;
-        const float v = ((float)(idx / kSunW) + 0.5f) / kSunH;
-        dir = equal_area_map_cone(sunDir, f3(P.sunT[0], P.sunT[1], P.sunT[2]), f3(P.sunB[0], P.sunB[1], P.sunB[2]), u,
-                                  v, P.cosThetaMax);
-        pdf = p * 1.0f;
-    }
+#endif
+
+struct LightFrame {
+    const float* skyCdf;
+    const float* sunCdf;
+    const float* lightSel;
+    F3 sunDir, sunT, sunB;
+    float cosThetaMax;
+#if !RTX_RNG_TABLES
+    const float* skyTree;
+    const float* sunTree;
+#endif
+};
+
+template <bool kSun, bool kHeaps>
+RT_DEV int light_search(const LightFrame& L, float target) {
+    const float* a = kSun ? L.sunCdf : L.skyCdf;
+    const int right = (kSun ? kSunSize : kSkySize) - 2;
+#if !RTX_RNG_TABLES
+    if constexpr (kHeaps)
+        return cdf_search_tree(a, right, target, kSun ? L.sunTree : L.skyTree, kSun ? kSunTreeNodes : kSkyTreeNodes);
+#endif
+    return cdf_search(a, 0, right, target);
+}
+
+template <bool kHeaps = false>
+RT_DEV void sample_light_sky(const LightFrame& L, float r0, F3& dir, float& pdf) {
+    const float pSky = L.lightSel[0], maxSky = L.lightSel[1];
+    const int idx = light_search<false, kHeaps>(L, r0 * maxSky) + 1;
+    float p = (L.skyCdf[idx] - L.skyCdf[idx - 1]) / maxSky;
+    p = div_two_pi(p * kSkySize);
+    const float u = ((float)(idx % kSkyW) + 0.5f) / kSkyW;
+    const float v = ((float)(idx / kSkyW) + 0.5f) / kSkyH;
+    dir = equal_area_map(u, v);
+    pdf = p * 1.0f * pSky;
+}
+template <bool kHeaps = false>
+RT_DEV void sample_light_sun(const LightFrame& L, float r0, F3& dir, float& pdf) {
+    const float maxSun = L.lightSel[2], sunDen = L.lightSel[3];
+    const int idx = light_search<true, kHeaps>(L, r0 * maxSun) + 1;
+    float p = (L.sunCdf[idx] - L.sunCdf[idx - 1]) / maxSun;
+    p = p * kSunSize / sunDen;
+    const float u = ((float)(idx % kSunW) + 0.5f) / kSunW;
+    const float v = ((float)(idx / kSunW) + 0.5f) / kSunH;
+    dir = equal_area_map_cone(L.sunDir, L.sunT, L.sunB, u, v, L.cosThetaMax);
+    pdf = p * 1.0f;
+}
+
+template <bool kHeaps = false>
+RT_DEV void sample_light(const LightFrame& L, F3& dir, float& pdf, int& lightIdx, float r0, float r1) {
+    if (L.lightSel[0] > r1) sample_light_sky<kHeaps>(L, r0, dir, pdf);
+    else sample_light_sun<kHeaps>(L, r0, dir, pdf);
     lightIdx = kEnvLightId;
 }
 
-RT_DEV void lambertian_sample(F2 u, F3& wo, F3 n) {
-    const float r = __builtin_sqrtf(u.x);
-    const float theta = kTwoPi * u.y;
-    const F2 d = {r * rt_cosf(theta), r * rt_sinf(theta)};
+constexpr int kLightTabSize = 512;
+RT_DEV void sample_light_table(const float4* lightTab, const float* lightSel, F3& dir, float& pdf, int& lightIdx, int b0,
+                               float r1) {
+    const float4 e = lightTab[2 * b0 + (lightSel[0] > r1 ? 0 : 1)];
+    dir = f3(e.x, e.y, e.z);
+    pdf = e.w;
+    lightIdx = kEnvLightId;
+}
+
+RT_DEV void lambertian_dir(float r, float cs, float sn, F3& wo, F3 n) {
+    const F2 d = {r * cs, r * sn};
     const float z = __builtin_sqrtf(max1f(0.0f, 1.0f - d.x * d.x - d.y * d.y));
     F3 uu, vv;
     localize_sample(n, uu, vv);
     wo = normalize(d.x * uu + d.y * vv + z * n);
+}
+RT_DEV void lambertian_sample(F2 u, F3& wo, F3 n) {
+    const float r = __builtin_sqrtf(u.x);
+    const float theta = kTwoPi * u.y;
+    lambertian_dir(r, rt_cosf(theta), rt_sinf(theta), wo, n);
 }
 
 RT_DEV F3 fresnel_schlick(F3 F0, float cosTheta) {
@@ -253,14 +296,17 @@
 
 RT_DEV F3 reflect3(F3 i, F3 n) { return i - 2.0f * n * dot(n, i); }
 
-RT_DEV F3 ggx_normal(F2 r, float alpha2, F3 normal) {
-    const float cosTheta = 1.0f / __builtin_sqrtf(1.0f + alpha2 * r.x / (1.0f - r.x));
+RT_DEV F3 ggx_normal_dir(float rx, float cs, float sn, float alpha2, F3 normal) {
+    const float cosTheta = 1.0f / __builtin_sqrtf(1.0f + alpha2 * rx / (1.0f - rx));
     const float sinTheta = __builtin_sqrtf(1.0f - cosTheta * cosTheta);
-    const float phi = kTwoPi * r.y;
-    const F3 sl = f3(sinTheta * rt_cosf(phi), cosTheta, sinTheta * rt_sinf(phi));
+    const F3 sl = f3(sinTheta * cs, cosTheta, sinTheta * sn);
     F3 t, b;
     localize_sample(normal, t, b);
     return normalize(sl.x * t + sl.z * b + sl.y * normal);
 }
-
-}
+RT_DEV F3 ggx_normal(F2 r, float alpha2, F3 normal) {
+    const float phi = kTwoPi * r.y;
+    return ggx_normal_dir(r.x, rt_cosf(phi), rt_sinf(phi), alpha2, normal);
+}
+
+}
diff --git a/real-time-ray-tracing_amd/csrc/sky.hip b/real-time-ray-tracing_amd/csrc/sky.hip
--- a/real-time-ray-tracing_amd/csrc/sky.hip
+++ b/real-time-ray-tracing_amd/csrc/sky.hip
@@ -162,6 +162,7 @@
     return rtk_launch_scan_ex(in, out, sums, size, blockSize, 1, stream);
 }
 
+#if !RTX_RNG_TABLES
 __global__ void k_cdf_tree(const float* cdf, int right0, float* tree, int nodes) {
     const int j = blockIdx.x * blockDim.x + threadIdx.x;
     if (j >= nodes) return;
@@ -177,6 +178,7 @@
     }
     tree[j] = live ? cdf[(left + right) / 2] : __builtin_nanf("");
 }
+#endif
 
 __global__ void k_light_select(const float* skyCdf, const float* sunCdf, float cosThetaMax, float* out) {
     const float maxSky = skyCdf[kSkySize - 1], maxSun = sunCdf[kSunSize - 1];
@@ -188,6 +190,39 @@
     out[3] = kTwoPi * (1.0f - cosThetaMax);
 }
 
+__global__ __launch_bounds__(kLightTabSize) void k_light_table(SkyGenParams P) {
+    const int b0 = (int)threadIdx.x >> 1;
+    LightFrame L{};
+    L.skyCdf = P.skyCdf;
+    L.sunCdf = P.sunCdf;
+    L.lightSel = P.lightSel;
+    L.sunDir = f3(P.sunDir[0], P.sunDir[1], P.sunDir[2]);
+    L.sunT = f3(P.sunT[0], P.sunT[1], P.sunT[2]);
+    L.sunB = f3(P.sunB[0], P.sunB[1], P.sunB[2]);
+    L.cosThetaMax = P.cosThetaMax;
+    F3 dir;
+    float pdf;
+    if ((threadIdx.x & 1u) == 0u) sample_light_sky(L, bn_float(b0), dir, pdf);
+    else sample_light_sun(L, bn_float(b0), dir, pdf);
+    P.lightTab[threadIdx.x] = make_float4(dir.x, dir.y, dir.z, pdf);
+}
+
+__global__ __launch_bounds__(256) void k_rng_tables(float2* lensDisk, float2* unitTrig, float* unitSqrt) {
+    const int i = (int)(blockIdx.x * 256u + threadIdx.x);
+    const F2 d = lens_disk<false>(nullptr, i >> 8, i & 255);
+    lensDisk[i] = make_float2(d.x, d.y);
+    if (i < 256) {
+        const float theta = kTwoPi * bn_float(i);
+        unitTrig[i] = make_float2(rt_cosf(theta), rt_sinf(theta));
+        unitSqrt[i] = __builtin_sqrtf(bn_float(i));
+    }
+}
+
+extern "C" hipError_t rtk_launch_rng_tables(float2* lensDisk, float2* unitTrig, float* unitSqrt, hipStream_t stream) {
+    hipLaunchKernelGGL(k_rng_tables, dim3(256), dim3(256), 0, stream, lensDisk, unitTrig, unitSqrt);
+    return hipGetLastError();
+}
+
 extern "C" hipError_t rtk_launch_sky(const SkyGenParams* p, hipStream_t stream) {
     hipLaunchKernelGGL(k_sky, dim3(kSkySize / 256), dim3(256), 0, stream, *p);
     hipError_t e = rtk_launch_scan(p->skyPdf, p->skyCdf, p->scanSums, kSkySize, kSkyScanBlock, stream);
@@ -195,11 +230,14 @@
     hipLaunchKernelGGL(k_sun, dim3(kSunSize / 256), dim3(256), 0, stream, *p);
     if ((e = rtk_launch_scan(p->sunPdf, p->sunCdf, p->scanSums, kSunSize, kSunScanBlock, stream)) != hipSuccess)
         return e;
+#if !RTX_RNG_TABLES
     hipLaunchKernelGGL(k_cdf_tree, dim3(kSkyTreeNodes / 256), dim3(256), 0, stream, p->skyCdf, kSkySize - 2,
                        p->skyTree, kSkyTreeNodes);
     hipLaunchKernelGGL(k_cdf_tree, dim3(kSunTreeNodes / 256), dim3(256), 0, stream, p->sunCdf, kSunSize - 2,
                        p->sunTree, kSunTreeNodes);
+#endif
     hipLaunchKernelGGL(k_light_select, dim3(1), dim3(1), 0, stream, (const float*)p->skyCdf, (const float*)p->sunCdf,
                        p->cosThetaMax, p->lightSel);
+    hipLaunchKernelGGL(k_light_table, dim3(1), dim3(kLightTabSize), 0, stream, *p);
     return hipGetLastError();
 }
diff --git a/real-time-ray-tracing_amd/csrc/trace_primary.hip b/real-time-ray-tracing_amd/csrc/trace_primary.hip
--- a/real-time-ray-tracing_amd/csrc/trace_primary.hip
+++ b/real-time-ray-tracing_amd/csrc/trace_primary.hip
@@ -21,10 +21,11 @@
 
     const int s = P.frameNum * 4 + 0;
     const F2 pix = {bluenoise(P.bluenoise, x, y, s, 0), bluenoise(P.bluenoise, x, y, s, 1)};
-    const F2 ap = {bluenoise(P.bluenoise, x, y, s, 2), bluenoise(P.bluenoise, x, y, s, 3)};
+    const F2 disk = lens_disk<kRngLensCamera>(P.lensDisk, bluenoise_byte(P.bluenoise, x, y, s, 2),
+                                              bluenoise_byte(P.bluenoise, x, y, s, 3));
     F3 org, dir, centerDir;
     F2 sampleUv;
-    generate_ray(P.cam, x, y, pix, ap, org, dir, centerDir, sampleUv);
+    generate_ray(P.cam, x, y, pix, disk, org, dir, centerDir, sampleUv);
 
     const SceneView sc = scene_view(P.nodes, P.tlasNodes, P.triPos, P.triNrm);
     HitInfo hi;
diff --git a/real-time-ray-tracing_amd/rtx/__init__.py b/real-time-ray-tracing_amd/rtx/__init__.py
--- a/real-time-ray-tracing_amd/rtx/__init__.py
+++ b/real-time-ray-tracing_amd/rtx/__init__.py
@@ -158,6 +158,7 @@
     "rt_sync": (C.c_int, [C.c_void_p]),
     "rt_time_stage": (C.c_int, [C.c_void_p, C.c_int, C.c_int, C.POINTER(C.c_float)]),
     "rt_debug_pk_math": (C.c_int, [C.c_int, C.c_void_p, C.c_float, C.c_float, C.c_void_p, C.c_void_p, C.c_size_t]),
+    "rt_debug_rng_tables": (C.c_int, [C.c_void_p, C.c_int, C.c_void_p, C.c_void_p, C.c_size_t]),
     "rt_time_path_trace_kernels": (C.c_int, [C.c_void_p, C.c_int, C.POINTER(C.c_float), C.c_int]),
     "rt_time_frame_kernels": (C.c_int, [C.c_void_p, C.c_int, C.c_int, C.POINTER(C.c_float), C.c_int]),
     "rt_trace_rays": (C.c_int, [C.c_void_p, C.c_void_p, C.c_uint32, C.c_void_p, C.c_void_p, C.POINTER(C.c_float)]),
@@ -599,6 +600,16 @@
                      QUERY_ANY_HIT if any_hit else 0, ready_event, done_event)
         self._check(self.lib.rt_trace_rays_device(self.h, C.byref(q)), "rt_trace_rays_device")
 
+    RNG_TABLES = dict(lensDisk=(0, (65536, 2)), unitTrig=(1, (256, 2)), unitSqrt=(2, (256,)), lightTab=(3, (256, 2, 4)),
+                      lightSel=(4, (4,)))
+
+    def debug_rng_tables(self, name: str):
+        which, shape = self.RNG_TABLES[name]
+        stored, direct = np.empty(shape, np.float32), np.empty(shape, np.float32)
+        self._check(self.lib.rt_debug_rng_tables(self.h, which, stored.ctypes.data, direct.ctypes.data, stored.nbytes),
+                    "rt_debug_rng_tables(%s)" % name)
+        return stored, direct
+
     def get_buffer(self, name: str, shape=None, dtype=np.uint8) -> np.ndarray:
         if shape is None:
             n = self.lib.rt_buffer_bytes(self.h, BUF[name])
```

After: 11720 Mray/s. 1.3% lower.
